# xxlong0/ESTDepth

Measured on AMD Instinct MI355X. Metric: depth frames/sec (seq_len=5, 480x640, D=64), higher is better.
Workload: dtype f32; 1 GPU; cfg2: seq_len=5, 480x640, ndepths=64, ResNet-50, Joint mode steady state (carried memory, EST on); launch=hipGraph replay, pipeline=False, graph_memory=zero-copy, conv3d_arith=f32, conv2d_arith=f32, conv3d_algo_32to32=wino3, full=False, parallelism=1 sequence per GPU

## Files before the change

### estdepth_amd/_native.py

```python
import ctypes
import os

_HERE = os.path.dirname(os.path.abspath(__file__))
LIB_PATH = os.environ.get("ESTD_LIB", os.path.join(_HERE, "lib", "libestd_hip.so"))

c_float_p = ctypes.c_void_p
c_stream = ctypes.c_void_p


class Conv3dDesc(ctypes.Structure):
    _fields_ = [
        ("N", ctypes.c_int), ("D", ctypes.c_int), ("H", ctypes.c_int), ("W", ctypes.c_int),
        ("cin_main", ctypes.c_int), ("in_stride", ctypes.c_int), ("n_tiles", ctypes.c_int),
        ("in_main", ctypes.c_void_p), ("in_extra", ctypes.c_void_p),
        ("w_main", ctypes.c_void_p), ("w_extra", ctypes.c_void_p), ("w_xout", ctypes.c_void_p),
        ("scale", ctypes.c_void_p), ("shift", ctypes.c_void_p),
        ("act_a", ctypes.c_int), ("act_b", ctypes.c_int), ("act_split", ctypes.c_int),
        ("out_main", ctypes.c_void_p), ("out_stride", ctypes.c_int), ("out_channels", ctypes.c_int),
        ("residual", ctypes.c_void_p), ("residual2", ctypes.c_void_p), ("out_scale", ctypes.c_float), ("accumulate", ctypes.c_int),
        ("out_extra", ctypes.c_void_p),
        ("head_w", ctypes.c_void_p), ("head_b", ctypes.c_void_p), ("out_head", ctypes.c_void_p),
        ("stats_partials", ctypes.c_void_p),
        ("w_split", ctypes.c_void_p),
        ("w_wino", ctypes.c_void_p),
# ... 16 lines not shown
        ("relu_before_residual", ctypes.c_int), ("relu_after_residual", ctypes.c_int),
        ("residual", ctypes.c_void_p), ("out", ctypes.c_void_p), ("w_split", ctypes.c_void_p), ("w_wino", ctypes.c_void_p),
    ]


class Conv1x1Desc(ctypes.Structure):
    _fields_ = [
        ("N", ctypes.c_int), ("H", ctypes.c_int), ("W", ctypes.c_int), ("cin", ctypes.c_int), ("cout", ctypes.c_int),
        ("stride", ctypes.c_int), ("relu", ctypes.c_int),
        ("in_", ctypes.c_void_p), ("w", ctypes.c_void_p), ("scale", ctypes.c_void_p), ("shift", ctypes.c_void_p),
        ("residual", ctypes.c_void_p), ("out", ctypes.c_void_p),
    ]


class Conv2dTapsDesc(ctypes.Structure):
    _fields_ = [
        ("N", ctypes.c_int), ("H", ctypes.c_int), ("W", ctypes.c_int), ("cin", ctypes.c_int), ("cout", ctypes.c_int),
        ("ksize", ctypes.c_int), ("stride", ctypes.c_int), ("pad", ctypes.c_int), ("relu", ctypes.c_int),
        ("in_", ctypes.c_void_p), ("w", ctypes.c_void_p), ("scale", ctypes.c_void_p), ("shift", ctypes.c_void_p),
        ("residual", ctypes.c_void_p), ("out", ctypes.c_void_p),
    ]


TSDF_MAX_FRAMES = 8
CONSISTENCY_MAX_SOURCES = 8


class TsdfIntegrateDesc(ctypes.Structure):
    _fields_ = [
        ("Z", ctypes.c_int), ("Y", ctypes.c_int), ("X", ctypes.c_int), ("T", ctypes.c_int), ("H", ctypes.c_int), ("W", ctypes.c_int),
        ("weighted", ctypes.c_int), ("no_skip", ctypes.c_int),
        ("trunc", ctypes.c_float), ("z_near", ctypes.c_float), ("conf_min", ctypes.c_float), ("w_max", ctypes.c_float),
        ("tsdf", ctypes.c_void_p), ("weight", ctypes.c_void_p),
        ("depth", ctypes.c_void_p * TSDF_MAX_FRAMES), ("conf", ctypes.c_void_p * TSDF_MAX_FRAMES), ("mats", (ctypes.c_float * 12) * TSDF_MAX_FRAMES),
    ]


class TsdfIntegrateColorDesc(ctypes.Structure):
    _fields_ = TsdfIntegrateDesc._fields_ + [("color", ctypes.c_void_p), ("image", ctypes.c_void_p * TSDF_MAX_FRAMES)]


class TsdfRaycastDesc(ctypes.Structure):
    _fields_ = [
        ("Z", ctypes.c_int), ("Y", ctypes.c_int), ("X", ctypes.c_int), ("H", ctypes.c_int), ("W", ctypes.c_int), ("n_steps", ctypes.c_int),
        ("t_min", ctypes.c_float), ("dt", ctypes.c_float), ("w_min", ctypes.c_float),
        ("tsdf", ctypes.c_void_p), ("weight", ctypes.c_void_p),
        ("depth", ctypes.c_void_p), ("normal", ctypes.c_void_p), ("out_weight", ctypes.c_void_p), ("stats", ctypes.c_void_p),
        ("mat", ctypes.c_float * 12),
    ]


class TsdfRaycastColorDesc(ctypes.Structure):
    _fields_ = TsdfRaycastDesc._fields_ + [("color", ctypes.c_void_p), ("out_color", ctypes.c_void_p)]


class DepthConsistencyDesc(ctypes.Structure):
    _fields_ = [
        ("H", ctypes.c_int), ("W", ctypes.c_int), ("S", ctypes.c_int),
        ("px_max", ctypes.c_float), ("rel_max", ctypes.c_float), ("z_near", ctypes.c_float),
        ("target", ctypes.c_void_p), ("source", ctypes.c_void_p * CONSISTENCY_MAX_SOURCES),
        ("views", ctypes.c_void_p), ("visible", ctypes.c_void_p), ("depth", ctypes.c_void_p), ("rel_err", ctypes.c_void_p),
        ("mats", ((ctypes.c_float * 12) * 2) * CONSISTENCY_MAX_SOURCES),
    ]


class CloudNearestDesc(ctypes.Structure):
    _fields_ = [
        ("M", ctypes.c_longlong), ("N", ctypes.c_longlong),
        ("query", ctypes.c_void_p), ("order", ctypes.c_void_p), ("records", ctypes.c_void_p), ("cell_start", ctypes.c_void_p),
        ("dist", ctypes.c_void_p), ("index", ctypes.c_void_p), ("stats", ctypes.c_void_p),
        ("lo", ctypes.c_float * 3), ("cell", ctypes.c_float), ("max_dist", ctypes.c_float), ("dims", ctypes.c_int * 3),
    ]


class MeshNearestDesc(ctypes.Structure):
    _fields_ = [
        ("M", ctypes.c_longlong), ("B", ctypes.c_longlong), ("P", ctypes.c_longlong),
        ("query", ctypes.c_void_p), ("order", ctypes.c_void_p), ("big_records", ctypes.c_void_p), ("records", ctypes.c_void_p),
        ("cell_start", ctypes.c_void_p), ("dist", ctypes.c_void_p), ("face", ctypes.c_void_p), ("bary", ctypes.c_void_p),
        ("closest", ctypes.c_void_p),
        ("lo", ctypes.c_float * 3), ("cell", ctypes.c_float), ("max_dist", ctypes.c_float), ("dims", ctypes.c_int * 3),
    ]


class FrameAlignDesc(ctypes.Structure):
    _fields_ = [
        ("H", ctypes.c_int), ("W", ctypes.c_int), ("Hm", ctypes.c_int), ("Wm", ctypes.c_int),
        ("dist_max", ctypes.c_float), ("z_near", ctypes.c_float), ("conf_min", ctypes.c_float),
        ("depth", ctypes.c_void_p), ("conf", ctypes.c_void_p), ("m_depth", ctypes.c_void_p), ("m_normal", ctypes.c_void_p),
        ("residual", ctypes.c_void_p), ("match", ctypes.c_void_p), ("sums", ctypes.c_void_p), ("partials", ctypes.c_void_p),
        ("L", ctypes.c_float * 12), ("Fm", ctypes.c_float * 12), ("Bm", ctypes.c_float * 12),
    ]


class RigidSystemDesc(ctypes.Structure):
    _fields_ = [
        ("N", ctypes.c_longlong), ("Nt", ctypes.c_longlong), ("Nn", ctypes.c_longlong),
        ("metric", ctypes.c_int), ("by_index", ctypes.c_int), ("two_sided", ctypes.c_int),
        ("dist_max", ctypes.c_float), ("cos_min", ctypes.c_float),
        ("moved", ctypes.c_void_p), ("moved_normal", ctypes.c_void_p), ("index", ctypes.c_void_p), ("target", ctypes.c_void_p),
        ("normal", ctypes.c_void_p), ("residual", ctypes.c_void_p), ("match", ctypes.c_void_p), ("sums", ctypes.c_void_p),
        ("partials", ctypes.c_void_p),
    ]


_SIGNATURES = {
    "estd_version": (ctypes.c_int, []),
    "estd_status_string": (ctypes.c_char_p, [ctypes.c_int]),
    "estd_profile_mark": (ctypes.c_int, [ctypes.c_int, c_stream]),
    "estd_set_reserved_cus": (ctypes.c_int, [ctypes.c_int]),
    "estd_get_reserved_cus": (ctypes.c_int, []),
    "estd_cam_pair_proj": (ctypes.c_int, [c_float_p, c_float_p, c_float_p, c_stream]),
    "estd_cam_sweep_proj": (ctypes.c_int, [c_float_p, c_float_p, c_float_p, c_float_p, c_stream]),
    "estd_cam_volume_mats": (ctypes.c_int, [c_float_p, c_float_p, c_float_p, c_float_p, c_stream]),
    "estd_homo_warping": (ctypes.c_int, [c_float_p, c_float_p, c_float_p, c_float_p,
                                         ctypes.c_int, ctypes.c_int, ctypes.c_int, ctypes.c_int, c_stream]),
    "estd_homo_warping_px": (ctypes.c_int, [c_float_p, c_float_p, c_float_p, c_float_p,
                                            ctypes.c_int, ctypes.c_int, ctypes.c_int, ctypes.c_int, c_stream]),
    "estd_warp_volume_ex": (ctypes.c_int, [c_float_p, c_float_p, c_float_p, ctypes.POINTER(WarpVolumeOpts), c_float_p,
                                           ctypes.c_int, ctypes.c_int, ctypes.c_int, ctypes.c_int, c_stream]),
    "estd_mix1x1_chw_to_hwc": (ctypes.c_int, [c_float_p, c_float_p, c_float_p, c_float_p,
                                              ctypes.c_int, ctypes.c_int, ctypes.c_int, c_stream]),
    "estd_homo_warp_costvol": (ctypes.c_int, [c_float_p, c_float_p, c_float_p, c_float_p, c_float_p,
                                              ctypes.c_int, ctypes.c_int, ctypes.c_int, c_stream]),
    "estd_conv3d_k3": (ctypes.c_int, [ctypes.POINTER(Conv3dDesc), c_stream]),
    "estd_conv3d_k3_split": (ctypes.c_int, [ctypes.POINTER(Conv3dDesc), c_stream]),
    "estd_conv3d_k3_wino": (ctypes.c_int, [ctypes.POINTER(Conv3dDesc), c_stream]),
    "estd_conv3d_k3_wino2": (ctypes.c_int, [ctypes.POINTER(Conv3dDesc), c_stream]),
    "estd_conv3d_k3_wino2x": (ctypes.c_int, [ctypes.POINTER(Conv3dDesc), c_stream]),
    "estd_conv3d_k3_wino3": (ctypes.c_int, [ctypes.POINTER(Conv3dDesc), c_stream]),
    "estd_conv3d_k3_xout": (ctypes.c_int, [ctypes.POINTER(Conv3dDesc), c_stream]),
    "estd_conv2d_k3": (ctypes.c_int, [ctypes.POINTER(Conv2dDesc), c_stream]),
    "estd_conv2d_k3_split": (ctypes.c_int, [ctypes.POINTER(Conv2dDesc), c_stream]),
    "estd_conv2d_k3_wino": (ctypes.c_int, [ctypes.POINTER(Conv2dDesc), c_stream]),
    "estd_conv2d_k3_wino2": (ctypes.c_int, [ctypes.POINTER(Conv2dDesc), c_stream]),
    "estd_conv3d_k3_grid": (ctypes.c_int, [ctypes.c_int, ctypes.c_int, ctypes.c_int, ctypes.c_int]),
    "estd_groupnorm_finalize": (ctypes.c_int, [c_float_p, ctypes.c_int, ctypes.c_double, ctypes.c_float,
                                               c_float_p, c_stream]),
    "estd_softargmin_up": (ctypes.c_int, [c_float_p, c_float_p, c_float_p, c_float_p,
                                          ctypes.c_int, ctypes.c_int, ctypes.c_int, ctypes.c_int, ctypes.c_int, c_stream]),
    "estd_warp_volume": (ctypes.c_int, [c_float_p, c_float_p, c_float_p, ctypes.c_float, ctypes.c_float, c_float_p,
                                        ctypes.c_int, ctypes.c_int, ctypes.c_int, ctypes.c_int, c_stream]),
    "estd_warp_attention": (ctypes.c_int, [c_float_p, ctypes.POINTER(ctypes.c_void_p), c_float_p, ctypes.c_int,
                                           c_float_p, ctypes.c_float, ctypes.c_float, c_float_p,
                                           ctypes.c_int, ctypes.c_int, ctypes.c_int, c_stream]),
    "estd_attention_prewarped": (ctypes.c_int, [c_float_p, ctypes.POINTER(ctypes.c_void_p), ctypes.c_int, c_float_p,
                                                ctypes.c_int64, c_stream]),
    "estd_gru_reset_apply": (ctypes.c_int, [c_float_p, c_float_p, c_float_p, c_float_p, c_float_p, c_float_p,
                                            ctypes.c_int64, c_stream]),
    "estd_gru_blend": (ctypes.c_int, [c_float_p] * 10 + [ctypes.c_int, ctypes.c_int64, c_stream]),
    "estd_bn_act_nhwc": (ctypes.c_int, [c_float_p, c_float_p, c_float_p, c_float_p, ctypes.c_int, ctypes.c_int64, ctypes.c_int, c_stream]),
    "estd_conv1x1_nhwc": (ctypes.c_int, [ctypes.POINTER(Conv1x1Desc), c_stream]),
    "estd_conv2d_taps_nhwc": (ctypes.c_int, [ctypes.POINTER(Conv2dTapsDesc), c_stream]),
    "estd_stem7x7s2_nhwc": (ctypes.c_int, [c_float_p, c_float_p, c_float_p, c_float_p, c_float_p, ctypes.c_int, ctypes.c_int, ctypes.c_int, c_stream]),
    "estd_maxpool3x3s2_nhwc": (ctypes.c_int, [c_float_p, c_float_p] + [ctypes.c_int] * 4 + [c_stream]),
    "estd_avgpool_nhwc": (ctypes.c_int, [c_float_p, c_float_p] + [ctypes.c_int] * 5 + [c_stream]),
    "estd_conv2d_small_nhwc": (ctypes.c_int, [c_float_p, c_float_p, c_float_p, c_float_p, c_float_p] + [ctypes.c_int] * 8 + [c_stream]),
    "estd_conv2d_k3_to16_nhwc": (ctypes.c_int, [c_float_p, c_float_p, c_float_p, c_float_p, c_float_p, ctypes.c_int, ctypes.c_int, ctypes.c_int,
                                                ctypes.c_int, ctypes.c_int, c_stream]),
    "estd_normalise_nhwc": (ctypes.c_int, [c_float_p, c_float_p, ctypes.c_int, ctypes.c_int64, c_stream]),
    "estd_stem3x3s2_nhwc": (ctypes.c_int, [c_float_p, c_float_p, c_float_p, c_float_p, c_float_p, ctypes.c_int, ctypes.c_int, ctypes.c_int, c_stream]),
    "estd_nhwc_to_planes": (ctypes.c_int, [c_float_p, ctypes.c_int, c_float_p, ctypes.c_int, ctypes.c_int64, c_stream]),
    "estd_planes_cat_nhwc": (ctypes.c_int, [c_float_p, ctypes.c_int, c_float_p, ctypes.c_int, ctypes.c_int, c_float_p, ctypes.c_int, ctypes.c_int64, c_stream]),
    "estd_upsample2_cat_nhwc": (ctypes.c_int, [c_float_p, ctypes.c_int, c_float_p, ctypes.c_int, c_float_p, ctypes.c_int, ctypes.c_int, ctypes.c_int, c_stream]),
    "estd_disp_head_nhwc": (ctypes.c_int, [c_float_p, c_float_p, c_float_p, ctypes.c_float, c_float_p, ctypes.c_int, ctypes.c_int, ctypes.c_int, ctypes.c_int,
                                           ctypes.c_int, c_stream]),
    "estd_spp_upsample_cat": (ctypes.c_int, [c_float_p, ctypes.c_int, c_float_p, ctypes.c_int, ctypes.POINTER(ctypes.c_void_p),
                                             ctypes.POINTER(ctypes.c_int), ctypes.POINTER(ctypes.c_int), ctypes.c_int, ctypes.c_int,
                                             c_float_p, ctypes.c_int, ctypes.c_int, ctypes.c_int, c_stream]),
    "estd_cdhw_to_vol": (ctypes.c_int, [c_float_p, c_float_p, ctypes.c_int, ctypes.c_int64, ctypes.c_int, ctypes.c_int, c_stream]),
    "estd_vol_to_cdhw": (ctypes.c_int, [c_float_p, c_float_p, ctypes.c_int, ctypes.c_int64, ctypes.c_int, ctypes.c_int, c_stream]),
    "estd_tsdf_integrate": (ctypes.c_int, [ctypes.POINTER(TsdfIntegrateDesc), c_stream]),
    "estd_tsdf_extract_points": (ctypes.c_int, [c_float_p, c_float_p, ctypes.c_int, ctypes.c_int, ctypes.c_int, ctypes.c_float,
                                                ctypes.POINTER(ctypes.c_float), ctypes.c_float, ctypes.c_void_p, ctypes.c_longlong,
                                                c_float_p, c_float_p, c_float_p, ctypes.c_void_p, c_stream]),
    "estd_tsdf_raycast": (ctypes.c_int, [ctypes.POINTER(TsdfRaycastDesc), c_stream]),
    "estd_tsdf_integrate_color": (ctypes.c_int, [ctypes.POINTER(TsdfIntegrateColorDesc), c_stream]),
    "estd_tsdf_edge_colors": (ctypes.c_int, [c_float_p, c_float_p, ctypes.c_int, ctypes.c_int, ctypes.c_int, ctypes.c_void_p, ctypes.c_longlong,
                                             c_float_p, c_stream]),
    "estd_tsdf_raycast_color": (ctypes.c_int, [ctypes.POINTER(TsdfRaycastColorDesc), c_stream]),
    "estd_depth_consistency": (ctypes.c_int, [ctypes.POINTER(DepthConsistencyDesc), c_stream]),
    "estd_cloud_cell_keys": (ctypes.c_int, [c_float_p, ctypes.c_longlong, ctypes.POINTER(ctypes.c_float), ctypes.c_float,
                                            ctypes.POINTER(ctypes.c_int), ctypes.c_void_p, c_stream]),
    "estd_cloud_nearest": (ctypes.c_int, [ctypes.POINTER(CloudNearestDesc), c_stream]),
    "estd_cloud_cell_centroids": (ctypes.c_int, [c_float_p, c_float_p, ctypes.c_int, ctypes.c_longlong, ctypes.c_void_p, ctypes.c_void_p,
                                                 ctypes.c_longlong, c_float_p, c_float_p, c_stream]),
    "estd_frame_align_partials": (ctypes.c_longlong, [ctypes.c_int, ctypes.c_int]),
    "estd_frame_align": (ctypes.c_int, [ctypes.POINTER(FrameAlignDesc), c_stream]),
    "estd_tsdf_mesh_vertices": (ctypes.c_int, [c_float_p, c_float_p, c_float_p, ctypes.c_int, ctypes.c_int, ctypes.c_int, ctypes.c_float,
                                               ctypes.POINTER(ctypes.c_float), ctypes.c_float, ctypes.c_void_p, ctypes.c_longlong,
                                               ctypes.c_void_p, c_float_p, c_float_p, c_float_p, c_float_p, c_stream]),
    "estd_tsdf_mesh_faces": (ctypes.c_int, [c_float_p, c_float_p, ctypes.c_int, ctypes.c_int, ctypes.c_int, ctypes.c_float, ctypes.c_void_p,
                                            ctypes.c_longlong, ctypes.c_void_p, ctypes.c_void_p, c_stream]),
    "estd_mesh_components": (ctypes.c_int, [ctypes.c_void_p, ctypes.c_longlong, ctypes.c_longlong, ctypes.c_void_p, ctypes.c_void_p,
                                            ctypes.c_void_p, c_stream]),
    "estd_mesh_face_area": (ctypes.c_int, [ctypes.c_void_p, ctypes.c_longlong, ctypes.c_void_p, ctypes.c_longlong, ctypes.c_void_p,
                                           ctypes.c_void_p, ctypes.c_void_p, c_stream]),
    "estd_mesh_sample": (ctypes.c_int, [ctypes.c_void_p, ctypes.c_longlong, ctypes.c_void_p, ctypes.c_longlong, ctypes.c_void_p, ctypes.c_int,
                                        ctypes.c_void_p, ctypes.c_void_p, ctypes.c_longlong, ctypes.c_longlong, ctypes.c_longlong,
                                        ctypes.c_ulonglong] + [ctypes.c_void_p] * 5 + [c_stream]),
    "estd_mesh_raster": (ctypes.c_int, [ctypes.c_void_p, ctypes.c_longlong, ctypes.c_void_p, ctypes.c_longlong, ctypes.c_longlong, ctypes.c_longlong,
                                        ctypes.POINTER(ctypes.c_double), ctypes.c_int, ctypes.c_int, ctypes.c_float, ctypes.c_int, ctypes.c_void_p,
                                        ctypes.c_void_p, c_stream]),
    "estd_mesh_raster_resolve": (ctypes.c_int, [ctypes.c_void_p, ctypes.c_longlong, ctypes.c_void_p, ctypes.c_longlong, ctypes.POINTER(ctypes.c_double),
                                                ctypes.c_int, ctypes.c_int] + [ctypes.c_void_p] * 5 + [c_stream]),
    "estd_mesh_tri_bins": (ctypes.c_int, [ctypes.c_void_p, ctypes.c_longlong, ctypes.c_void_p, ctypes.c_longlong, ctypes.POINTER(ctypes.c_float),
                                          ctypes.c_float, ctypes.POINTER(ctypes.c_int), ctypes.c_int, ctypes.c_void_p, ctypes.c_void_p,
                                          ctypes.c_void_p, c_stream]),
    "estd_mesh_tri_fill": (ctypes.c_int, [ctypes.c_void_p, ctypes.c_longlong, ctypes.c_void_p, ctypes.c_longlong, ctypes.POINTER(ctypes.c_float),
                                          ctypes.c_float, ctypes.POINTER(ctypes.c_int), ctypes.c_int, ctypes.c_void_p, ctypes.c_longlong,
                                          ctypes.c_void_p, ctypes.c_void_p, c_stream]),
    "estd_mesh_nearest": (ctypes.c_int, [ctypes.POINTER(MeshNearestDesc), c_stream]),
    "estd_mesh_cluster_faces": (ctypes.c_int, [ctypes.c_void_p, ctypes.c_longlong, ctypes.c_longlong, ctypes.c_void_p, ctypes.c_longlong,
                                               ctypes.c_void_p, ctypes.c_void_p, ctypes.c_void_p, c_stream]),
    "estd_mesh_cluster_quadrics": (ctypes.c_int, [ctypes.c_void_p, ctypes.c_longlong, ctypes.c_void_p, ctypes.c_longlong, ctypes.c_void_p,
                                                  ctypes.c_void_p, ctypes.c_void_p, ctypes.c_longlong, ctypes.c_void_p,
                                                  ctypes.POINTER(ctypes.c_float), ctypes.c_float, ctypes.POINTER(ctypes.c_int), ctypes.c_double,
                                                  ctypes.c_void_p, ctypes.c_void_p, ctypes.c_void_p, c_stream]),
    "estd_rigid_apply": (ctypes.c_int, [ctypes.c_void_p, ctypes.c_void_p, ctypes.c_longlong, ctypes.POINTER(ctypes.c_float), ctypes.c_void_p,
                                        ctypes.c_void_p, c_stream]),
    "estd_rigid_system_partials": (ctypes.c_longlong, [ctypes.c_longlong]),
    "estd_rigid_system": (ctypes.c_int, [ctypes.POINTER(RigidSystemDesc), c_stream]),
}

AB_SYMBOLS = ("estd_conv3d_k3_split", "estd_conv3d_k3_wino", "estd_conv2d_k3_split", "estd_conv2d_k3_wino", "estd_conv3d_k3_wino2x")
EXPORTED_SYMBOLS = tuple(k for k in _SIGNATURES if k not in AB_SYMBOLS)

_lib = None


def lib():
    global _lib
    if _lib is None:
        if not os.path.exists(LIB_PATH):
            raise RuntimeError("libestd_hip.so not found at %s -- build it with `python -m estdepth_amd.build` "
                               "(there is no CPU/eager fallback)" % LIB_PATH)
        handle = ctypes.CDLL(LIB_PATH)
        for name, (res, args) in _SIGNATURES.items():
            if name in AB_SYMBOLS and not hasattr(handle, name):
                continue
            fn = getattr(handle, name)
            fn.restype = res
            fn.argtypes = args
        _lib = handle
    return _lib


def has_ab():
    return all(hasattr(lib(), n) for n in AB_SYMBOLS)


def require_ab(what):
    if not has_ab():
        raise RuntimeError("%s needs the A/B kernels: rebuild the library with ESTD_BUILD_AB=1 (python -m estdepth_amd.build)" % what)


def check(status, what):
    if status != 0:
        msg = lib().estd_status_string(status).decode()
        raise RuntimeError("%s failed: %s (estd_status %d)" % (what, msg, status))
```

### estdepth_amd/backbones.py

```python
import os

import numpy as np
import torch
import torch.nn as nn
import torch.nn.functional as F


SPP_FUSED = os.environ.get("ESTD_SPP_FUSED", "1") == "1"


def conv_bn2d(cin, cout, k, stride, pad, dilation):
    return nn.Sequential(
        nn.Conv2d(cin, cout, k, stride, dilation if dilation > 1 else pad, dilation, bias=False),
        nn.BatchNorm2d(cout))


def _folded(bn):
    from . import packing
    key = (bn.weight.device, bn.weight._version, bn.bias._version, bn.running_mean._version, bn.running_var._version,
           bn.weight.data_ptr())
    c = bn.__dict__.get("_estd_fold")
    if c is None or c[0] != key:
        sc, sh = packing.fold_bn_fp32(bn, list(range(bn.num_features)))
        c = (key, sc.to(bn.weight.device), sh.to(bn.weight.device))
        bn.__dict__["_estd_fold"] = c
    return c[1], c[2]


def fused_on(mod, x):
    return mod.__dict__.get("_fuse_bn", False) and x.is_cuda and not mod.training


def conv1x1_gemm(conv, x):
    key = (conv.weight.device, conv.weight._version, conv.weight.data_ptr())
    c = conv.__dict__.get("_estd_w2")
    if c is None or c[0] != key:
        c = (key, conv.weight.detach().reshape(conv.out_channels, conv.in_channels).t().contiguous())
        conv.__dict__["_estd_w2"] = c
    if conv.stride != (1, 1):
        x = x[:, :, ::conv.stride[0], ::conv.stride[1]]
    x = x.contiguous(memory_format=torch.channels_last)
    n, cin, h, w = x.shape
    y = torch.mm(x.permute(0, 2, 3, 1).reshape(n * h * w, cin), c[1])
    if conv.bias is not None:
        y = y + conv.bias
    return y.view(n, h, w, conv.out_channels).permute(0, 3, 1, 2)


HIP_STEM = os.environ.get("ESTD_HIP_STEM", "1") == "1"
HIP_STEM7 = os.environ.get("ESTD_HIP_STEM7", "1") == "1"
HIP_POOL = os.environ.get("ESTD_HIP_POOL", "1") == "1"
GEMM_EPILOGUE = os.environ.get("ESTD_GEMM_EPILOGUE", "1") == "1"
HIP_1X1 = os.environ.get("ESTD_HIP_1X1", "all")


def _hip_1x1_wanted(conv, residual):
    if HIP_1X1 == "all" or HIP_1X1 == "1":
        return True
    if HIP_1X1 != "auto":
        return False
    return residual is not None or (conv.stride == (2, 2) and conv.in_channels <= 512) or (conv.in_channels <= 64 and conv.out_channels <= 64)


def conv1x1_bn_gemm(conv, bn, x, relu):
    key = (conv.weight.device, conv.weight._version, conv.weight.data_ptr(), bn.weight._version, bn.bias._version,
           bn.running_mean._version, bn.running_var._version)
    c = conv.__dict__.get("_estd_w2bn")
    if c is None or c[0] != key:
        sc, sh = _folded(bn)
        w2 = conv.weight.detach().reshape(conv.out_channels, conv.in_channels).t() * sc[None, :]
        c = (key, w2.contiguous(), sh.contiguous())
        conv.__dict__["_estd_w2bn"] = c
    if conv.stride != (1, 1):
        x = x[:, :, ::conv.stride[0], ::conv.stride[1]]
    x = x.contiguous(memory_format=torch.channels_last)
    n, cin, h, w = x.shape
    x2 = x.permute(0, 2, 3, 1).reshape(n * h * w, cin)
    y = torch._addmm_activation(c[2], x2, c[1], use_gelu=False) if relu else torch.addmm(c[2], x2, c[1])
    return y.view(n, h, w, conv.out_channels).permute(0, 3, 1, 2)


HIP_TAPS = os.environ.get("ESTD_HIP_TAPS", "1") == "1"


def _fits_32bit(x, conv):
    n, _, h, w = x.shape
    ho, wo = (h + conv.stride[0] - 1) // conv.stride[0], (w + conv.stride[1] - 1) // conv.stride[1]
    return max(n * h * w * conv.in_channels, n * ho * wo * conv.out_channels) * 4 < 0x7fffff00


def _hip_taps_ok(conv):
    k = conv.kernel_size[0]
    return HIP_TAPS and conv.kernel_size == (k, k) and k in (3, 5) and conv.stride in ((1, 1), (2, 2)) and conv.dilation == (1, 1) \
        and conv.groups == 1 and conv.bias is None and conv.padding[0] == conv.padding[1] and conv.in_channels % 16 == 0 \
        and conv.out_channels % 32 == 0 and conv.weight.is_cuda and conv.padding_mode == "zeros"


def _is_1x1(conv):
    return conv.kernel_size == (1, 1) and conv.padding == (0, 0) and conv.groups == 1 and conv.dilation == (1, 1)


HIP_3X3_MIN_ITEMS = int(os.environ.get("ESTD_HIP3X3_MIN_ITEMS", "128"))


def _hip_3x3_plan(conv, bn, x, relu, has_residual):
    if not conv.__dict__.get("_hip3x3", False) or conv.kernel_size != (3, 3) or conv.stride != (1, 1) or conv.groups != 1:
        return None
    if conv.bias is not None or conv.dilation not in ((1, 1), (2, 2)) or conv.padding != conv.dilation:
        return None
    if conv.in_channels % 32 or conv.out_channels % 32:
        return None
    n, _, h, w = x.shape
    if n * ((h + 7) // 8) * ((w + 15) // 16) * (conv.out_channels // 32) < HIP_3X3_MIN_ITEMS:
        return None
    from . import ops
    key = (conv.weight.device, conv.weight._version, conv.weight.data_ptr(), bn.weight._version, bn.bias._version,
           bn.running_mean._version, bn.running_var._version, relu, has_residual)
    c = conv.__dict__.get("_estd_plan3x3")
    if c is None or c[0] != key:
        c = (key, ops.Conv2dPlan(conv, bn, relu_before=relu and not has_residual, relu_after=relu and has_residual))
        conv.__dict__["_estd_plan3x3"] = c
    return c[1]


def enable_hip_3x3(root, enable=True):
    for m in root.modules():
        if isinstance(m, nn.Conv2d):
            m.__dict__["_hip3x3"] = bool(enable)
    return root


def conv_bn_act(conv, bn, x, relu, residual=None):
    from . import ops
    plan = _hip_3x3_plan(conv, bn, x, relu, residual is not None)
    if plan is not None:
        xn = x.contiguous(memory_format=torch.channels_last).permute(0, 2, 3, 1)
        rn = residual.contiguous(memory_format=torch.channels_last).permute(0, 2, 3, 1) if residual is not None else None
        return plan.run(xn, residual=rn).permute(0, 3, 1, 2)
    if _is_1x1(conv) and conv.bias is None and conv.stride in ((1, 1), (2, 2)) and conv.in_channels % 16 == 0 \
            and conv.out_channels % 32 == 0 and _hip_1x1_wanted(conv, residual) and _fits_32bit(x, conv):
        key = (conv.weight.device, conv.weight._version, conv.weight.data_ptr())
        c = conv.__dict__.get("_estd_w1x1")
        if c is None or c[0] != key:
            c = (key, conv.weight.detach().reshape(conv.out_channels, conv.in_channels).contiguous())
            conv.__dict__["_estd_w1x1"] = c
        sc, sh = _folded(bn)
        xn = x.contiguous(memory_format=torch.channels_last).permute(0, 2, 3, 1)
        rn = residual.contiguous(memory_format=torch.channels_last).permute(0, 2, 3, 1) if residual is not None else None
        return ops.conv1x1_nhwc(xn, c[1], sc, sh, conv.stride[0], relu, rn).permute(0, 3, 1, 2)
    if _hip_taps_ok(conv) and _fits_32bit(x, conv):
        from . import packing
        key = (conv.weight.device, conv.weight._version, conv.weight.data_ptr())
        c = conv.__dict__.get("_estd_wtaps")
        if c is None or c[0] != key:
            c = (key, packing.pack_conv2d_taps(conv.weight).to(conv.weight.device))
            conv.__dict__["_estd_wtaps"] = c
        sc, sh = _folded(bn)
        xn = x.contiguous(memory_format=torch.channels_last).permute(0, 2, 3, 1)
        rn = residual.contiguous(memory_format=torch.channels_last).permute(0, 2, 3, 1) if residual is not None else None
        return ops.conv2d_taps_nhwc(xn, c[1], sc, sh, conv.kernel_size[0], conv.stride[0], conv.padding[0], relu, rn).permute(0, 3, 1, 2)
    if GEMM_EPILOGUE and residual is None and _is_1x1(conv) and conv.bias is None:
        return conv1x1_bn_gemm(conv, bn, x, relu)
    y = conv1x1_gemm(conv, x) if _is_1x1(conv) else conv(x)
    if not y.is_contiguous(memory_format=torch.channels_last):
        y = y.contiguous(memory_format=torch.channels_last)
    if residual is not None and not residual.is_contiguous(memory_format=torch.channels_last):
        residual = residual.contiguous(memory_format=torch.channels_last)
    sc, sh = _folded(bn)
    return ops.bn_act_nhwc_(y, sc, sh, relu, residual)


HIP_SMALL = os.environ.get("ESTD_HIP_SMALL_CONVS", "1") == "1"


def small_conv_nhwc(conv, bn, x_nhwc, relu):
    from . import ops, packing
    k, s = conv.kernel_size[0], conv.stride[0]
    if not HIP_SMALL or conv.bias is not None or conv.groups != 1 or conv.dilation != (1, 1) or conv.kernel_size != (k, k) \
            or conv.stride != (s, s) or conv.padding != (k // 2, k // 2) or (conv.in_channels, k, s) not in ops.SMALL_CONV_SHAPES \
            or conv.out_channels % 16 or not x_nhwc.is_cuda:
        return None
    key = (conv.weight.device, conv.weight._version, conv.weight.data_ptr()) + \
        ((bn.weight._version, bn.bias._version, bn.running_mean._version, bn.running_var._version) if bn is not None else ())
    c = conv.__dict__.get("_estd_small")
    if c is None or c[0] != key:
        dev = conv.weight.device
        if bn is not None:
            sc, sh = _folded(bn)
        else:
            sc, sh = torch.ones(conv.out_channels, device=dev), torch.zeros(conv.out_channels, device=dev)
        c = (key, packing.pack_conv2d_small(conv.weight).to(dev), sc.float().contiguous(), sh.float().contiguous())
        conv.__dict__["_estd_small"] = c
    return ops.conv2d_small_nhwc(x_nhwc.contiguous(), c[1], c[2], c[3], conv.out_channels, k, s, relu)


def enable_fused_bn(root, enable=True):
    for m in root.modules():
        if isinstance(m, (_PSMBlock, PSMFeatures, _Basic, _Bottleneck, SemanticEncoder, UpBlock)):
            m.__dict__["_fuse_bn"] = bool(enable)
    return root


class _PSMBlock(nn.Module):
    def __init__(self, cin, cout, stride, downsample, pad, dilation):
        super().__init__()
        self.conv1 = nn.Sequential(conv_bn2d(cin, cout, 3, stride, pad, dilation), nn.ReLU(inplace=True))
        self.conv2 = conv_bn2d(cout, cout, 3, 1, pad, dilation)
        self.downsample = downsample

    def shortcut(self, x):
        if self.downsample is None:
            return x
        if fused_on(self, x):
            return conv_bn_act(self.downsample[0], self.downsample[1], x, relu=False)
        return self.downsample(x)

    def first(self, x):
        if fused_on(self, x):
            return conv_bn_act(self.conv1[0][0], self.conv1[0][1], x, relu=True)
        return self.conv1(x)

    def forward(self, x):
        if fused_on(self, x):
            return conv_bn_act(self.conv2[0], self.conv2[1], self.first(x), relu=False, residual=self.shortcut(x))
        y = self.conv2(self.conv1(x))
        return y + (x if self.downsample is None else self.downsample(x))


class PSMFeatures(nn.Module):

    def __init__(self):
        super().__init__()
        self._cin = 32
        self.firstconv = nn.Sequential(
            conv_bn2d(3, 32, 3, 2, 1, 1), nn.ReLU(inplace=True),
            conv_bn2d(32, 32, 3, 1, 1, 1), nn.ReLU(inplace=True),
            conv_bn2d(32, 32, 3, 1, 1, 1), nn.ReLU(inplace=True))
        self.layer1 = self._stage(32, 3, 1, 1, 1)
        self.layer2 = self._stage(64, 16, 2, 1, 1)
        self.layer3 = self._stage(128, 3, 1, 1, 1)
        self.layer4 = self._stage(128, 3, 1, 1, 2)
        for i, p in zip((1, 2, 3, 4), (32, 16, 8, 4)):
            setattr(self, "branch%d" % i, nn.Sequential(
                nn.AvgPool2d((p, p), stride=(p, p)), conv_bn2d(128, 32, 1, 1, 0, 1), nn.ReLU(inplace=True)))
        self.lastconv = nn.Sequential(conv_bn2d(320, 128, 3, 1, 1, 1), nn.ReLU(inplace=True),
                                      nn.Conv2d(128, 32, 1, 1, 0, bias=False))
        self.out_channels = [32]

    def _stage(self, planes, blocks, stride, pad, dilation):
        down = None
        if stride != 1 or self._cin != planes:
            down = nn.Sequential(nn.Conv2d(self._cin, planes, 1, stride, bias=False), nn.BatchNorm2d(planes))
        layers = [_PSMBlock(self._cin, planes, stride, down, pad, dilation)]
        self._cin = planes
        layers += [_PSMBlock(planes, planes, 1, None, pad, dilation) for _ in range(1, blocks)]
        return nn.Sequential(*layers)

    def use_hip_convs(self, enable=True):
        self._hip = bool(enable)
        self._hip_plans = None
        if enable:
            self.to(memory_format=torch.channels_last)
        return self

    def _plans(self):
        from . import ops
        key = tuple((p.data_ptr(), p._version) for p in self.parameters())
        if getattr(self, "_hip_plans", None) is None or self._hip_plans[0] != key:
            plans = {}
            fc = self.firstconv
            plans["first1"] = ops.Conv2dPlan(fc[2][0], fc[2][1], relu_before=True)
            plans["first2"] = ops.Conv2dPlan(fc[4][0], fc[4][1], relu_before=True)
            for lname in ("layer1", "layer2", "layer3", "layer4"):
                for bi, blk in enumerate(getattr(self, lname)):
                    c1 = blk.conv1[0]
                    if c1[0].stride == (1, 1):
                        plans[(lname, bi, 1)] = ops.Conv2dPlan(c1[0], c1[1], relu_before=True)
                    plans[(lname, bi, 2)] = ops.Conv2dPlan(blk.conv2[0], blk.conv2[1])
            plans["last"] = ops.Conv2dPlan(self.lastconv[0][0], self.lastconv[0][1], relu_before=True)
            self._hip_plans = (key, plans)
        return self._hip_plans[1]

    @staticmethod
    def _nhwc(t):
        return t.contiguous(memory_format=torch.channels_last).permute(0, 2, 3, 1)

    @staticmethod
    def _nchw(t):
        return t.permute(0, 3, 1, 2)

    def _forward_hip(self, x):
        P = self._plans()
        fc = self.firstconv
        x = x.contiguous(memory_format=torch.channels_last)
        c0 = fc[0][0]
        if HIP_STEM and c0.in_channels == 3 and c0.out_channels == 32 and c0.kernel_size == (3, 3) and c0.stride == (2, 2) \
                and c0.padding == (1, 1) and c0.dilation == (1, 1) and c0.bias is None:
            from . import ops
            key = (c0.weight.data_ptr(), c0.weight._version, c0.weight.device)
            cw = c0.__dict__.get("_estd_w_nchw")
            if cw is None or cw[0] != key:
                cw = (key, c0.weight.detach().contiguous(memory_format=torch.contiguous_format).clone())
                c0.__dict__["_estd_w_nchw"] = cw
            sc, sh = _folded(fc[0][1])
            x = ops.stem3x3s2_nhwc(self._nhwc(x), cw[1], sc, sh)
        else:
            x = conv_bn_act(c0, fc[0][1], x, relu=True) if fused_on(self, x) else fc[1](fc[0](x))
            x = self._nhwc(x)
        x = P["first2"].run(P["first1"].run(x))
        for lname in ("layer1", "layer2", "layer3", "layer4"):
            for bi, blk in enumerate(getattr(self, lname)):
                if (lname, bi, 1) in P:
                    y = P[(lname, bi, 1)].run(x)
# ... 240 lines not shown
```

### estdepth_amd/build.py

```python
import os
import subprocess
import sys
from concurrent.futures import ThreadPoolExecutor

HERE = os.path.dirname(os.path.abspath(__file__))
ROOT = os.path.dirname(HERE)
CSRC = os.path.join(HERE, "csrc")
OUT_DIR = os.path.join(HERE, "lib")
OBJ_DIR = os.path.join(OUT_DIR, "obj" + os.environ.get("ESTD_LIB_SUFFIX", ""))
LIB = os.path.join(OUT_DIR, "libestd_hip%s.so" % os.environ.get("ESTD_LIB_SUFFIX", ""))
SOURCES = ["conv3d_mfma.hip", "conv3d_wino2.hip", "conv3d_wino3.hip", "conv3d_xout.hip", "conv3d_wino2_c16.hip", "conv2d_mfma.hip", "conv2d_wino2.hip",
           "plane_sweep.hip", "est_fusion.hip", "refine2d.hip", "conv1x1.hip", "conv2d_taps.hip", "tsdf.hip", "tsdf_raycast.hip",
           "depth_consistency.hip", "cloud_nn.hip", "track/frame_align.hip", "track/rigid_align.hip",
           "mesh/tsdf_mesh.hip", "mesh/mesh_components.hip",
           "mesh/mesh_sample.hip", "mesh/mesh_raster.hip", "mesh/mesh_distance.hip", "mesh/mesh_simplify.hip"]
AB_SOURCES = ["conv3d_wino.hip", "conv3d_split_bf16.hip", "conv2d_wino.hip", "conv2d_split_bf16.hip", "conv3d_wino2x.hip"]
BUILD_AB = os.environ.get("ESTD_BUILD_AB", "0") == "1"
if BUILD_AB:
    SOURCES = SOURCES + AB_SOURCES
HEADERS = [os.path.join(ROOT, "include", "estd_hip.h"), os.path.join(CSRC, "estd_common.h"), os.path.join(CSRC, "estd_device.h")]
FLAGS = ["--offload-arch=gfx950", "-O3", "-std=c++17", "-fPIC",
         "-I" + os.path.join(ROOT, "include"), "-I" + CSRC] + (["-DESTD_BUILD_AB=1"] if BUILD_AB else [])
MODE_STAMP = os.path.join(OUT_DIR, ".build_mode" + os.environ.get("ESTD_LIB_SUFFIX", ""))


def _hipcc():
    for c in (os.environ.get("HIPCC"), "/opt/rocm/bin/hipcc", "hipcc"):
        if c and (os.path.isabs(c) and os.path.exists(c) or not os.path.isabs(c)):
            return c
    return "hipcc"


def _stale(target, deps):
    if not os.path.exists(target):
        return True
    t = os.path.getmtime(target)
    return any(os.path.getmtime(d) > t for d in deps)


def build(force=False, verbose=False):
    os.makedirs(OBJ_DIR, exist_ok=True)
    hipcc = _hipcc()
    mode = "ab" if BUILD_AB else "default"
    relink = (open(MODE_STAMP).read().strip() if os.path.exists(MODE_STAMP) else "default" if os.path.exists(LIB) else "") != mode
    jobs = []
    objs = []
    for src in SOURCES:
        s = os.path.join(CSRC, src)
        o = os.path.join(OBJ_DIR, src.replace(".hip", ".o"))
        os.makedirs(os.path.dirname(o), exist_ok=True)
        objs.append(o)
        if force or _stale(o, [s] + HEADERS):
            cmd = [hipcc] + FLAGS + os.environ.get("ESTD_BUILD_DEFS", "").split() + (["-Rpass-analysis=kernel-resource-usage"] if verbose else []) + ["-c", s, "-o", o]
            jobs.append(cmd)

    def run(cmd):
        r = subprocess.run(cmd, capture_output=True, text=True)
        if r.returncode != 0:
            raise RuntimeError("hipcc failed: %s\n%s" % (" ".join(cmd), r.stderr))
        return r.stderr

    if jobs:
        with ThreadPoolExecutor(max_workers=len(jobs)) as ex:
            for log in ex.map(run, jobs):
                if verbose and log:
                    sys.stderr.write(log)
    if force or jobs or relink or _stale(LIB, objs):
        run([hipcc, "--offload-arch=gfx950", "-shared", "-fPIC"] + objs + ["-o", LIB])
    build_torch_ops(force=force or relink)
    open(MODE_STAMP, "w").write(mode)
    return LIB


TORCH_OPS_SRC = os.path.join(CSRC, "torch_ops.cpp")
TORCH_OPS_LIB = os.path.join(OUT_DIR, "libestd_torch_ops%s.so" % os.environ.get("ESTD_LIB_SUFFIX", ""))


def build_torch_ops(force=False):
    if not (force or _stale(TORCH_OPS_LIB, [TORCH_OPS_SRC, HEADERS[0], LIB])):
        return TORCH_OPS_LIB
    import torch
    from torch.utils import cpp_extension
    tlib = os.path.join(os.path.dirname(torch.__file__), "lib")
    cmd = [_hipcc(), "-O2", "-std=c++17", "-fPIC", "-shared", "-D__HIP_PLATFORM_AMD__=1", "-DUSE_ROCM=1", "-DHIPBLAS_V2",
           "-D_GLIBCXX_USE_CXX11_ABI=%d" % int(torch._C._GLIBCXX_USE_CXX11_ABI), "-I" + os.path.join(ROOT, "include")] \
        + (["-DESTD_BUILD_AB=1"] if BUILD_AB else [])
    cmd += ["-I" + p for p in cpp_extension.include_paths("cuda")]
    cmd += [TORCH_OPS_SRC, "-o", TORCH_OPS_LIB, "-L" + OUT_DIR, "-l:" + os.path.basename(LIB), "-L" + tlib,
            "-lc10", "-lc10_hip", "-ltorch_cpu", "-ltorch_hip", "-ltorch", "-Wl,-rpath,$ORIGIN", "-Wl,-rpath," + tlib]
    r = subprocess.run(cmd, capture_output=True, text=True)
    if r.returncode != 0:
        raise RuntimeError("hipcc failed: %s\n%s" % (" ".join(cmd), r.stderr[-4000:]))
    return TORCH_OPS_LIB


if __name__ == "__main__":
    print(build(force="--force" in sys.argv, verbose="--verbose" in sys.argv))
```

### estdepth_amd/csrc/conv2d_taps.hip

```cpp
#include <hip/hip_runtime.h>
#include <stdint.h>
#include <stdlib.h>

#include "estd_hip.h"
#include "estd_common.h"
#include "estd_device.h"

namespace {

template <int TM, int TN, int PF, int SK>
__global__ __launch_bounds__(256) void conv2d_taps_kernel(const estd_conv2d_taps_desc p, int Ho, int Wo, int tiles_m, int tiles_n)
{
    __shared__ float4 red[SK > 1 ? (SK - 1) * TN * TM * 64 : 1];
    const int lane = threadIdx.x & 63;
    const int wave = __builtin_amdgcn_readfirstlane(threadIdx.x >> 6);
    const int g = lane >> 4, i = lane & 15;
    const int wt = SK > 1 ? (int)blockIdx.x : (int)blockIdx.x * 4 + wave;
    if (wt >= tiles_m * tiles_n) return;
    const int tn = wt % tiles_n, tm = wt / tiles_n;
    const int m0 = tm * 16 * TM, n0 = tn * 16 * TN;
    const int Mtot = p.N * Ho * Wo;
    const int cin = p.cin, cout = p.cout, ks = p.ksize;

    const __amdgpu_buffer_rsrc_t rs_x = make_rsrc_bytes(p.in, (size_t)p.N * p.H * p.W * cin * 4);
    const __amdgpu_buffer_rsrc_t rs_w = make_rsrc_bytes(p.w, (size_t)ks * ks * cout * cin * 4);
    int xbase[TM];
    unsigned xmask[TM], woff[TN];
#pragma unroll
    for (int t = 0; t < TM; ++t) {
        const int m = m0 + 16 * t + i;
        const int x = m % Wo, r = m / Wo;
        const int y = r % Ho, n = r / Ho;
        const int y0 = y * p.stride - p.pad, x0 = x * p.stride - p.pad;
        xbase[t] = (((n * p.H + y0) * p.W + x0) * cin + 4 * g) * 4;
        unsigned mk = 0;
        if (m < Mtot)
            for (int ky = 0; ky < ks; ++ky)
                for (int kx = 0; kx < ks; ++kx)
                    if ((unsigned)(y0 + ky) < (unsigned)p.H && (unsigned)(x0 + kx) < (unsigned)p.W) mk |= 1u << (ky * ks + kx);
        xmask[t] = mk;
    }
#pragma unroll
    for (int t = 0; t < TN; ++t) woff[t] = (unsigned)((n0 + 16 * t + i) * cin + 4 * g) * 4u;

    f32x4 acc[TN][TM];
#pragma unroll
    for (int a = 0; a < TN; ++a)
#pragma unroll
        for (int b = 0; b < TM; ++b) acc[a][b] = (f32x4){0.f, 0.f, 0.f, 0.f};

    const int cpt = cin >> 4;
    const int nchunks = ks * ks * cpt / SK;
    const int kbase = SK > 1 ? wave * nchunks : 0;
    int l_tap = kbase / cpt, l_kc = kbase - l_tap * cpt;
    int l_ky = l_tap / ks, l_kx = l_tap - l_ky * ks;

    float4 xq[PF][TM], wq[PF][TN];
    auto load_next = [&](float4 (&xd)[TM], float4 (&wd)[TN]) {
        const int xdelta = ((l_ky * p.W + l_kx) * cin + l_kc * 16) * 4;
        const int wdelta = (l_tap * cout * cin + l_kc * 16) * 4;
#pragma unroll
        for (int t = 0; t < TN; ++t) wd[t] = as_float4(__builtin_amdgcn_raw_buffer_load_b128(rs_w, woff[t], wdelta, 0));
#pragma unroll
        for (int t = 0; t < TM; ++t) {
            const unsigned off = ((xmask[t] >> l_tap) & 1u) ? (unsigned)(xbase[t] + xdelta) : OOB_OFFSET;
            xd[t] = as_float4(__builtin_amdgcn_raw_buffer_load_b128(rs_x, off, 0, 0));
        }
        if (++l_kc == cpt) {
            l_kc = 0; ++l_tap;
            if (++l_kx == ks) { l_kx = 0; ++l_ky; }
        }
    };
    auto mfma_chunk = [&](const float4 (&xs)[TM], const float4 (&ws)[TN]) {
#pragma unroll
        for (int e = 0; e < 4; ++e)
#pragma unroll
            for (int a = 0; a < TN; ++a) {
                const float wv = e == 0 ? ws[a].x : e == 1 ? ws[a].y : e == 2 ? ws[a].z : ws[a].w;
#pragma unroll
                for (int b = 0; b < TM; ++b) {
                    const float xv = e == 0 ? xs[b].x : e == 1 ? xs[b].y : e == 2 ? xs[b].z : xs[b].w;
                    acc[a][b] = __builtin_amdgcn_mfma_f32_16x16x4f32(wv, xv, acc[a][b], 0, 0, 0);
                }
            }
    };
#pragma unroll
    for (int j = 0; j < PF - 1; ++j)
        if (j < nchunks) load_next(xq[j], wq[j]);
    for (int c = 0; c < nchunks; c += PF) {
#pragma unroll
        for (int j = 0; j < PF; ++j) {
            const int cc = c + j;
            if (cc + PF - 1 < nchunks) load_next(xq[(j + PF - 1) % PF], wq[(j + PF - 1) % PF]);
            if (cc < nchunks) mfma_chunk(xq[j], wq[j]);
        }
    }
    if (SK > 1) {
        if (wave > 0) {
#pragma unroll
            for (int a = 0; a < TN; ++a)
#pragma unroll
                for (int b = 0; b < TM; ++b)
                    red[(((wave - 1) * TN + a) * TM + b) * 64 + lane] = make_float4(acc[a][b][0], acc[a][b][1], acc[a][b][2], acc[a][b][3]);
        }
        __syncthreads();
        if (wave > 0) return;
#pragma unroll
        for (int w = 0; w < SK - 1; ++w)
#pragma unroll
            for (int a = 0; a < TN; ++a)
#pragma unroll
                for (int b = 0; b < TM; ++b) {
                    const float4 r = red[((w * TN + a) * TM + b) * 64 + lane];
                    acc[a][b] += (f32x4){r.x, r.y, r.z, r.w};
                }
    }

    const __amdgpu_buffer_rsrc_t rs_o = make_rsrc_bytes(p.out, (size_t)Mtot * cout * 4);
    const __amdgpu_buffer_rsrc_t rs_r = make_rsrc_bytes(p.residual ? p.residual : p.out, (size_t)Mtot * cout * 4);
    const float floor_ = p.relu ? 0.0f : ESTD_NO_FLOOR;
#pragma unroll
    for (int a = 0; a < TN; ++a) {
        const int cb = n0 + 16 * a + 4 * g;
        float4 sc = make_float4(1.f, 1.f, 1.f, 1.f), sh = make_float4(0.f, 0.f, 0.f, 0.f);
        if (p.scale) sc = *reinterpret_cast<const float4*>(p.scale + cb);
        if (p.shift) sh = *reinterpret_cast<const float4*>(p.shift + cb);
        unsigned ooff[TM];
        float4 res[TM];
#pragma unroll
        for (int b = 0; b < TM; ++b) {
            const int m = m0 + 16 * b + i;
            ooff[b] = m < Mtot ? (unsigned)((size_t)m * cout + cb) * 4u : OOB_OFFSET;
        }
        if (p.residual) {
#pragma unroll
            for (int b = 0; b < TM; ++b) res[b] = as_float4(__builtin_amdgcn_raw_buffer_load_b128(rs_r, ooff[b], 0, 0));
        }
#pragma unroll
        for (int b = 0; b < TM; ++b) {
            float4 v;
            v.x = fmaf(acc[a][b][0], sc.x, sh.x); v.y = fmaf(acc[a][b][1], sc.y, sh.y);
            v.z = fmaf(acc[a][b][2], sc.z, sh.z); v.w = fmaf(acc[a][b][3], sc.w, sh.w);
            if (p.residual) { v.x += res[b].x; v.y += res[b].y; v.z += res[b].z; v.w += res[b].w; }
            v.x = fmaxf(v.x, floor_); v.y = fmaxf(v.y, floor_); v.z = fmaxf(v.z, floor_); v.w = fmaxf(v.w, floor_);
            u32x4 bits;
            __builtin_memcpy(&bits, &v, 16);
            __builtin_amdgcn_raw_buffer_store_b128(bits, rs_o, ooff[b], 0, 0);
        }
    }
}

template <int TM, int TN, int PF, int SK>
int launch_taps(const estd_conv2d_taps_desc& d, int Ho, int Wo, hipStream_t stream)
{
    const long long Mtot = (long long)d.N * Ho * Wo;
    const int tiles_m = (int)((Mtot + 16 * TM - 1) / (16 * TM)), tiles_n = d.cout / (16 * TN);
    const long long wts = (long long)tiles_m * tiles_n;
    const unsigned grid = SK > 1 ? (unsigned)wts : (unsigned)((wts + 3) / 4);
    hipLaunchKernelGGL((conv2d_taps_kernel<TM, TN, PF, SK>), dim3(grid), dim3(256), 0, stream, d, Ho, Wo, tiles_m, tiles_n);
    return ESTD_LAUNCH_CHECK();
}

constexpr int STEM_ROWS = 8;
__global__ __launch_bounds__(256) void stem7x7s2_nhwc_kernel(const float* __restrict__ in, const float* __restrict__ wpk, const float* __restrict__ scale,
                                                             const float* __restrict__ shift, float* __restrict__ out, int N, int H, int W, int Ho,
                                                             int Wo, int strips_y, int segs_x)
{
    const int lane = threadIdx.x & 63, g = lane >> 4, i = lane & 15;
    const long long wid = (long long)blockIdx.x * 4 + (threadIdx.x >> 6);
    const long long nwaves = (long long)N * strips_y * segs_x;
    if (wid >= nwaves) return;
    const int seg = (int)(wid % segs_x);
    const int strip = (int)((wid / segs_x) % strips_y);
    const int n = (int)(wid / ((long long)segs_x * strips_y));

    float wr[7][6][4];
#pragma unroll
    for (int ky = 0; ky < 7; ++ky)
#pragma unroll
        for (int s = 0; s < 6; ++s)
#pragma unroll
            for (int u = 0; u < 4; ++u) wr[ky][s][u] = wpk[((ky * 6 + s) * 4 + u) * 64 + lane];
    float4 sc[4], sh[4];
#pragma unroll
    for (int u = 0; u < 4; ++u) {
        sc[u] = reinterpret_cast<const float4*>(scale + 16 * u)[g];
        sh[u] = reinterpret_cast<const float4*>(shift + 16 * u)[g];
    }
    const __amdgpu_buffer_rsrc_t rs_in =
        __builtin_amdgcn_make_buffer_rsrc(const_cast<float*>(in + (size_t)n * H * W * 3), 0, (int)((size_t)H * W * 3 * 4), 0x00020000);
    const int x = seg * 16 + i;
    const int c0 = 2 * x - 3 + 2 * g, c1 = c0 + 1;
    const unsigned off0 = (x < Wo && (unsigned)c0 < (unsigned)W) ? (unsigned)c0 * 12u : OOB_OFFSET;
    const unsigned off1 = (x < Wo && g < 3 && (unsigned)c1 < (unsigned)W) ? (unsigned)c1 * 12u : OOB_OFFSET;
    for (int r = 0; r < STEM_ROWS; ++r) {
        const int y = strip * STEM_ROWS + r;
        if (y >= Ho) break;
        f32x4 acc[4];
#pragma unroll
        for (int u = 0; u < 4; ++u) acc[u] = (f32x4){0.f, 0.f, 0.f, 0.f};
#pragma unroll
        for (int ky = 0; ky < 7; ++ky) {
            const int yy = 2 * y - 3 + ky;
            if ((unsigned)yy >= (unsigned)H) continue;
            const int rowoff = yy * W * 12;
            const u32x3 r0 = __builtin_amdgcn_raw_buffer_load_b96(rs_in, off0, rowoff, 0);
            const u32x3 r1 = __builtin_amdgcn_raw_buffer_load_b96(rs_in, off1, rowoff, 0);
            float a[6];
            __builtin_memcpy(&a[0], &r0, 12);
            __builtin_memcpy(&a[3], &r1, 12);
#pragma unroll
            for (int s = 0; s < 6; ++s)
#pragma unroll
                for (int u = 0; u < 4; ++u) acc[u] = __builtin_amdgcn_mfma_f32_16x16x4f32(wr[ky][s][u], a[s], acc[u], 0, 0, 0);
        }
        if (x < Wo) {
#pragma unroll
            for (int u = 0; u < 4; ++u) {
                float4 o;
                o.x = fmaxf(fmaf(acc[u][0], sc[u].x, sh[u].x), 0.f);
                o.y = fmaxf(fmaf(acc[u][1], sc[u].y, sh[u].y), 0.f);
                o.z = fmaxf(fmaf(acc[u][2], sc[u].z, sh[u].z), 0.f);
                o.w = fmaxf(fmaf(acc[u][3], sc[u].w, sh[u].w), 0.f);
                *reinterpret_cast<float4*>(out + (((size_t)n * Ho + y) * Wo + x) * 64 + 16 * u + 4 * g) = o;
            }
        }
    }
}

__global__ __launch_bounds__(256) void maxpool3x3s2_nhwc_kernel(const float4* __restrict__ in, float4* __restrict__ out, int N, int H, int W, int C4,
                                                                int Ho, int Wo, long long total)
{
    const long long e = (long long)blockIdx.x * 256 + threadIdx.x;
    if (e >= total) return;
    const int c = (int)(e % C4);
    const long long pix = e / C4;
    const int x = (int)(pix % Wo), y = (int)((pix / Wo) % Ho);
    const long long n = pix / ((long long)Wo * Ho);
    const float ninf = -__builtin_inff();
    float4 m = make_float4(ninf, ninf, ninf, ninf);
#pragma unroll
    for (int ky = 0; ky < 3; ++ky) {
        const int yy = 2 * y - 1 + ky;
        if ((unsigned)yy >= (unsigned)H) continue;
#pragma unroll
        for (int kx = 0; kx < 3; ++kx) {
            const int xx = 2 * x - 1 + kx;
            if ((unsigned)xx >= (unsigned)W) continue;
            const float4 v = in[((n * H + yy) * W + xx) * C4 + c];
            m.x = (v.x > m.x || v.x != v.x) ? v.x : m.x;
            m.y = (v.y > m.y || v.y != v.y) ? v.y : m.y;
            m.z = (v.z > m.z || v.z != v.z) ? v.z : m.z;
            m.w = (v.w > m.w || v.w != v.w) ? v.w : m.w;
        }
    }
    out[e] = m;
}

__global__ __launch_bounds__(256) void avgpool_nhwc_kernel(const float4* __restrict__ in, float4* __restrict__ out, int H, int W, int C4, int k,
                                                           int Ho, int Wo, long long total)
{
    const long long e = (long long)blockIdx.x * 256 + threadIdx.x;
    if (e >= total) return;
    const int c = (int)(e % C4);
    const long long pix = e / C4;
    const int x = (int)(pix % Wo), y = (int)((pix / Wo) % Ho);
    const long long n = pix / ((long long)Wo * Ho);
    float4 s = make_float4(0.f, 0.f, 0.f, 0.f);
    for (int ky = 0; ky < k; ++ky) {
        const float4* row = in + ((n * H + (long long)y * k + ky) * W + (long long)x * k) * C4 + c;
        for (int kx = 0; kx < k; ++kx) {
            const float4 v = row[(long long)kx * C4];
            s.x += v.x; s.y += v.y; s.z += v.z; s.w += v.w;
        }
    }
    const float div = (float)(k * k);
    out[e] = make_float4(s.x / div, s.y / div, s.z / div, s.w / div);
}

}

extern "C" int estd_conv2d_taps_nhwc(const estd_conv2d_taps_desc* dp, estd_stream_t s)
{
    if (!dp) return ESTD_ERR_ARG;
    const estd_conv2d_taps_desc& d = *dp;
    if (d.N <= 0 || d.H <= 0 || d.W <= 0 || !d.in || !d.w || !d.out || d.pad < 0) return ESTD_ERR_ARG;
    if (d.stride != 1 && d.stride != 2) return ESTD_ERR_UNSUPPORTED;
    if (d.ksize != 1 && d.ksize != 3 && d.ksize != 5) return ESTD_ERR_UNSUPPORTED;
    if (d.cin < 16 || (d.cin & 15) || d.cout < 32 || (d.cout & 31)) return ESTD_ERR_UNSUPPORTED;
    if (d.H + 2 * d.pad < d.ksize || d.W + 2 * d.pad < d.ksize) return ESTD_ERR_ARG;
    const int Ho = (d.H + 2 * d.pad - d.ksize) / d.stride + 1, Wo = (d.W + 2 * d.pad - d.ksize) / d.stride + 1;
    const long long Mtot = (long long)d.N * Ho * Wo;
    const int taps = d.ksize * d.ksize;
    if (((long long)d.N * d.H + d.ksize) * d.W * d.cin * 4 >= 0x7fffff00LL || Mtot * d.cout * 4 >= 0x7fffff00LL ||
        (long long)taps * d.cin * d.cout * 4 >= 0x7fffff00LL)
        return ESTD_ERR_UNSUPPORTED;
    hipStream_t stream = estd_stream(s);
    static const int cfg_env = [] { const char* e = getenv("ESTD_CTAPS_CFG"); return e ? atoi(e) : 0; }();
    const long long want = (long long)estd_device_cus() * 7 / 2;
    auto tiles = [&](int tm, int tn) { return ((Mtot + 16 * tm - 1) / (16 * tm)) * (d.cout / (16 * tn)); };
    const bool sk4 = (d.cin & 63) == 0 && (long long)taps * d.cin >= 256;
    const bool c64 = (d.cout & 63) == 0;
    int cfg = cfg_env;
    if (cfg == 0) {
        if (c64 && tiles(4, 4) >= want) cfg = 441;
        else if (tiles(4, 2) >= want) cfg = 421;
        else if (sk4 && c64 && tiles(4, 4) >= want / 4) cfg = 444;
        else if (tiles(2, 2) >= want) cfg = 221;
        else if (sk4 && c64 && tiles(2, 4) >= want / 4) cfg = 244;
        else if (sk4 && tiles(2, 2) >= want / 4) cfg = 224;
        else if (sk4) cfg = 124;
        else cfg = 121;
    }
    if ((cfg % 10) == 4 && (d.cin & 63)) cfg = cfg - 3;
    if ((cfg / 10) % 10 == 4 && !c64) cfg -= 20;
    switch (cfg) {
    case 441: return launch_taps<4, 4, 2, 1>(d, Ho, Wo, stream);
    case 421: return launch_taps<4, 2, 3, 1>(d, Ho, Wo, stream);
    case 241: return launch_taps<2, 4, 3, 1>(d, Ho, Wo, stream);
    case 221: return launch_taps<2, 2, 4, 1>(d, Ho, Wo, stream);
    case 444: return launch_taps<4, 4, 2, 4>(d, Ho, Wo, stream);
    case 424: return launch_taps<4, 2, 3, 4>(d, Ho, Wo, stream);
    case 244: return launch_taps<2, 4, 3, 4>(d, Ho, Wo, stream);
    case 224: return launch_taps<2, 2, 4, 4>(d, Ho, Wo, stream);
    case 124: return launch_taps<1, 2, 4, 4>(d, Ho, Wo, stream);
    default: return launch_taps<1, 2, 8, 1>(d, Ho, Wo, stream);
    }
}

extern "C" int estd_stem7x7s2_nhwc(const float* in, const float* w_packed, const float* scale, const float* shift, float* out, int N, int H, int W,
                                   estd_stream_t s)
{
    if (!in || !w_packed || !scale || !shift || !out || N <= 0 || H <= 0 || W <= 0) return ESTD_ERR_ARG;
    if ((long long)H * W * 12 >= 0x7fffff00LL) return ESTD_ERR_UNSUPPORTED;
    const int Ho = (H - 1) / 2 + 1, Wo = (W - 1) / 2 + 1;
    const int strips_y = (Ho + STEM_ROWS - 1) / STEM_ROWS, segs_x = (Wo + 15) / 16;
    const long long waves = (long long)N * strips_y * segs_x;
    const long long blocks = (waves + 3) / 4;
    if (blocks > 0x7fffffffLL) return ESTD_ERR_ARG;
    hipLaunchKernelGGL(stem7x7s2_nhwc_kernel, dim3((unsigned)blocks), dim3(256), 0, estd_stream(s), in, w_packed, scale, shift, out, N, H, W, Ho, Wo,
                       strips_y, segs_x);
    return ESTD_LAUNCH_CHECK();
}

extern "C" int estd_maxpool3x3s2_nhwc(const float* in, float* out, int N, int H, int W, int C, estd_stream_t s)
{
    if (!in || !out || N <= 0 || H <= 0 || W <= 0 || C <= 0 || (C & 3)) return ESTD_ERR_ARG;
    const int Ho = (H - 1) / 2 + 1, Wo = (W - 1) / 2 + 1;
    const long long total = (long long)N * Ho * Wo * (C / 4);
    const long long blocks = (total + 255) / 256;
    if (blocks > 0x7fffffffLL) return ESTD_ERR_ARG;
    hipLaunchKernelGGL(maxpool3x3s2_nhwc_kernel, dim3((unsigned)blocks), dim3(256), 0, estd_stream(s), reinterpret_cast<const float4*>(in),
                       reinterpret_cast<float4*>(out), N, H, W, C / 4, Ho, Wo, total);
    return ESTD_LAUNCH_CHECK();
}

extern "C" int estd_avgpool_nhwc(const float* in, float* out, int N, int H, int W, int C, int k, estd_stream_t s)
{
    if (!in || !out || N <= 0 || H <= 0 || W <= 0 || C <= 0 || (C & 3) || k <= 0 || k > H || k > W) return ESTD_ERR_ARG;
    const int Ho = H / k, Wo = W / k;
    const long long total = (long long)N * Ho * Wo * (C / 4);
    const long long blocks = (total + 255) / 256;
    if (blocks > 0x7fffffffLL) return ESTD_ERR_ARG;
    hipLaunchKernelGGL(avgpool_nhwc_kernel, dim3((unsigned)blocks), dim3(256), 0, estd_stream(s), reinterpret_cast<const float4*>(in),
                       reinterpret_cast<float4*>(out), H, W, C / 4, k, Ho, Wo, total);
    return ESTD_LAUNCH_CHECK();
}
```

### estdepth_amd/csrc/estd_common.h

```cpp
#ifndef ESTD_COMMON_H
#define ESTD_COMMON_H

#include <hip/hip_runtime.h>

#include "estd_hip.h"

#define ESTD_LAUNCH_CHECK() (hipGetLastError() == hipSuccess ? ESTD_OK : ESTD_ERR_LAUNCH)

static inline hipStream_t estd_stream(estd_stream_t s) { return static_cast<hipStream_t>(s); }

#define ESTD_NO_FLOOR __builtin_nanf("")

extern "C" int estd_get_reserved_cus(void);
#include <atomic>
#include <stdio.h>
static inline int estd_device_cus(void)
{
    static std::atomic<int> cus[64];
    int dev = 0;
    if (hipGetDevice(&dev) != hipSuccess) dev = 0;
    int n = 0;
    const bool cached = (unsigned)dev < 64u;
    if (cached && (n = cus[dev].load(std::memory_order_relaxed)) > 0) return n;
    if (hipDeviceGetAttribute(&n, hipDeviceAttributeMultiprocessorCount, dev) != hipSuccess || n <= 0) {
        static std::atomic<bool> warned{false};
        if (!warned.exchange(true))
            fprintf(stderr, "libestd_hip: hipDeviceGetAttribute(MultiprocessorCount) failed for device %d: persistent grids sized for 256 CUs\n", dev);
        return 256;
    }
    if (cached) cus[dev].store(n, std::memory_order_relaxed);
    return n;
}
static inline int estd_persistent_wgs(int per_cu)
{
    const int cus = estd_device_cus() - estd_get_reserved_cus();
    return (cus > 8 ? cus : 8) * per_cu;
}
static inline int estd_persistent_grid(long long total, int per_cu)
{
    const int slots = estd_persistent_wgs(per_cu);
    int grid = total < slots ? (int)total : slots;
    if (grid >= 8) grid &= ~7;
    return grid;
}

static inline bool estd_conv3d_volume_fits_rsrc(const estd_conv3d_desc& d)
{
    const long long vox = (long long)d.D * d.H * d.W;
    const int widest = d.in_stride > d.out_stride ? d.in_stride : d.out_stride;
    return vox * widest * 4 < 0x7fffff00LL;
}

static inline int estd_conv3d_readback_kind(bool res_any, bool accumulate)
{
    return (!res_any && !accumulate) ? 0 : (!res_any ? 1 : (!accumulate ? 2 : 3));
}

static inline bool finite_pos(float v) { return v > 0.f && v < __builtin_inff(); }

int estd_wino2_c16_launch(const estd_conv3d_desc& d, hipStream_t stream);

static inline int estd_ceil_div(long long a, long long b) { return (int)((a + b - 1) / b); }

template <auto Kernel>
static inline void estd_allow_dynamic_lds(int bytes)
{
    static std::atomic<unsigned long long> done{0ull};
    int dev = 0;
    if (hipGetDevice(&dev) != hipSuccess) dev = 0;
    const unsigned long long bit = 1ull << (dev & 63);
    if (!(done.load(std::memory_order_acquire) & bit)) {
        (void)hipFuncSetAttribute(reinterpret_cast<const void*>(Kernel), hipFuncAttributeMaxDynamicSharedMemorySize, bytes);
        done.fetch_or(bit, std::memory_order_release);
    }
}

#endif
```

### estdepth_amd/csrc/torch_ops.cpp

```cpp
#include <ATen/ATen.h>
#include <ATen/hip/HIPContext.h>
#include <ATen/DeviceGuard.h>
#include <c10/hip/HIPStream.h>
#include <torch/library.h>

#include <algorithm>
#include <cmath>
#include <string>
#include <type_traits>
#include <vector>

#include "estd_hip.h"

namespace {

using at::Tensor;
using OptTensor = std::optional<Tensor>;

inline estd_stream_t cur_stream() { return static_cast<estd_stream_t>(c10::hip::getCurrentHIPStream().stream()); }

struct OpScope {
    static inline thread_local const c10::Device* cur = nullptr;
    c10::OptionalDeviceGuard guard;
    c10::Device dev;
// ... 906 lines not shown
static const int32_t* check_clusters(const Tensor& cluster, int64_t n_clusters, const Tensor& faces, const char* op)
{
    const int32_t* c = lptr<int32_t>(cluster, op, "cluster", faces, -1);
    check_count(cluster.size(0), 0, 0x7fffffffLL, op, "the number of vertices");
    check_count(n_clusters, cluster.size(0) ? 1 : 0, cluster.size(0), op, "n_clusters");
    return c;
}

std::tuple<Tensor, Tensor, Tensor> mesh_cluster_faces(const Tensor& faces, const Tensor& cluster, int64_t n_clusters)
{
    const char* op = "mesh_cluster_faces";
    const int32_t* f = faces_ptr(faces, op, "faces");
    const OpScope scope(faces);
    const int32_t* c = check_clusters(cluster, n_clusters, faces, op);
    const int64_t F = faces.size(0), V = cluster.size(0);
    TORCH_CHECK(F <= 0x7fffffffLL / 3, op, ": at most ", 0x7fffffffLL / 3, " faces, got ", F);
    Tensor corner = at::empty({3 * F}, faces.options()), triple = at::empty({F, 3}, faces.options());
    Tensor counts = at::empty({2}, faces.options().dtype(at::kLong));
    check_status(estd_mesh_cluster_faces(F ? f : nullptr, (long long)F, (long long)V, V ? c : nullptr, (long long)n_clusters,
                                         F ? corner.data_ptr<int32_t>() : nullptr, F ? triple.data_ptr<int32_t>() : nullptr,
                                         reinterpret_cast<long long*>(counts.data_ptr<int64_t>()), cur_stream()), "estd_mesh_cluster_faces");
    if (F && !n_clusters) {
        corner.zero_();
        triple.fill_(-1);
        counts.select(0, 0).fill_(F);
    }
    return {corner, triple, counts};
}

std::tuple<Tensor, Tensor, Tensor> mesh_cluster_quadrics(const Tensor& xyz, const Tensor& faces, const Tensor& order, const Tensor& segments,
                                                         const Tensor& cell_key, const Tensor& mean, const Tensor& lo, double cell,
                                                         at::IntArrayRef dims, double reg)
{
    const char* op = "mesh_cluster_quadrics";
    const OpScope scope(faces);
    const MeshArg m = check_mesh(xyz, faces, op);
    TORCH_CHECK(m.F <= 0x7fffffffLL / 3, op, ": at most ", 0x7fffffffLL / 3, " faces, got ", m.F);
    const int64_t* ord = lptr(order, op, "order", faces, 3 * m.F);
    const int64_t* seg = lptr(segments, op, "segments", faces, -1);
    TORCH_CHECK(segments.size(0) >= 1 && segments.size(0) <= m.V + 1, op, ": segments must be [K + 1] with K <= ", m.V, " vertices");
    const int64_t K = segments.size(0) - 1;
    const int64_t* key = lptr(cell_key, op, "cell_key", faces, K);
    const float* mu = check_cloud(mean, op, "mean", 3);
    TORCH_CHECK(mean.size(0) == K && mean.device() == faces.device(), op, ": mean must be [", K, ",3] on the faces' device");
    check_cloud_grid(lo, cell, dims, op, ESTD_CLOUD_KEY_MAX_DIM);
    TORCH_CHECK(std::isfinite(reg) && reg >= 0, op, ": reg must be finite and not negative, got ", reg);
    Tensor out = new_f32({K, 3}, xyz), normal = new_f32({K, 3}, xyz), placed = at::empty({K}, faces.options().dtype(at::kBool));
    const int d3[3] = {(int)dims[0], (int)dims[1], (int)dims[2]};
    check_status(estd_mesh_cluster_quadrics(m.V ? m.xyz : nullptr, (long long)m.V, m.F ? m.faces : nullptr, (long long)m.F,
                                            m.F ? reinterpret_cast<const long long*>(ord) : nullptr, reinterpret_cast<const long long*>(seg),
                                            K ? reinterpret_cast<const long long*>(key) : nullptr, (long long)K, K ? mu : nullptr,
                                            lo.data_ptr<float>(), (float)cell, d3, reg, K ? out.data_ptr<float>() : nullptr,
                                            K ? normal.data_ptr<float>() : nullptr,
                                            K ? reinterpret_cast<unsigned char*>(placed.data_ptr<bool>()) : nullptr, cur_stream()),
                 "estd_mesh_cluster_quadrics");
    if (K && !m.F) {
        out.copy_(mean);
        normal.zero_();
        placed.zero_();
    }
    return {out, normal, placed};
}

Tensor warp_attention(const Tensor& kv_target, at::TensorList kv_sources, const Tensor& mats, const Tensor& depth_values,
                      double depth_min, double depth_interval)
{
    const char* op = "warp_attention";
    const OpScope scope(kv_target);
    const float* kv = map_ptr(kv_target, {-1, -1, -1, 32}, op, "kv_target");
    const int64_t D = kv_target.size(-4), H = kv_target.size(-3), W = kv_target.size(-2), n = (int64_t)kv_sources.size();
    check_count(n, 1, ESTD_MAX_ATTENTION_SOURCES, op, "kv_sources");
    const std::vector<const float*> srcs = like_ptrs(kv_sources, kv_target, op, "kv_sources");
    const float* m = floats_ptr(mats, n * 30, op, "mats");
    const float* dv = floats_ptr(depth_values, D, op, "depth_values", true);
    Tensor xh = at::empty_like(kv_target);
    ESTD_LAUNCH(estd_warp_attention, kv, srcs.data(), m, (int)n, dv, (float)depth_min, (float)depth_interval, xh.data_ptr<float>(), (int)D, (int)H,
                (int)W);
    return xh;
}

Tensor attention_prewarped(const Tensor& kv_target, at::TensorList kv_sources)
{
    const char* op = "attention_prewarped";
    const OpScope scope(kv_target);
    const int64_t n_vox = records(kv_target, op, "kv_target"), n = (int64_t)kv_sources.size();
    check_count(n, 1, ESTD_MAX_ATTENTION_SOURCES, op, "kv_sources");
    const std::vector<const float*> srcs = like_ptrs(kv_sources, kv_target, op, "kv_sources");
    Tensor xh = at::empty_like(kv_target);
    ESTD_LAUNCH(estd_attention_prewarped, kv_target.data_ptr<float>(), srcs.data(), (int)n, xh.data_ptr<float>(), n_vox);
    return xh;
}

Tensor gru_reset_apply(const Tensor& xh, const Tensor& ru, const Tensor& stats4, const Tensor& gamma_r, const Tensor& beta_r)
{
    const char* op = "gru_reset_apply";
    const OpScope scope(xh);
    const int64_t n_vox = records(xh, op, "xh");
    const float *x = xh.data_ptr<float>(), *r = floats_ptr(ru, n_vox * 32, op, "ru");
    const float *st = floats_ptr(stats4, 4, op, "stats4"), *ga = floats_ptr(gamma_r, 16, op, "gamma_r"), *be = floats_ptr(beta_r, 16, op, "beta_r");
    Tensor xrh = at::empty_like(xh);
    ESTD_LAUNCH(estd_gru_reset_apply, x, r, st, ga, be, xrh.data_ptr<float>(), n_vox);
    return xrh;
}

void gru_blend(const Tensor& xh, const Tensor& ru, const Tensor& o_raw, const Tensor& stats_ru, const Tensor& stats_o,
               const Tensor& gamma_u, const Tensor& beta_u, const Tensor& gamma_o, const Tensor& beta_o, Tensor out_value, int64_t out_stride)
{
    const char* op = "gru_blend";
    const OpScope scope(xh);
    const int64_t n_vox = records(xh, op, "xh");
    const float *x = xh.data_ptr<float>(), *r = floats_ptr(ru, n_vox * 32, op, "ru"), *o = floats_ptr(o_raw, n_vox * 16, op, "o_raw");
    const float *sr = floats_ptr(stats_ru, 4, op, "stats_ru"), *so = floats_ptr(stats_o, 4, op, "stats_o");
    const float *gu = floats_ptr(gamma_u, 16, op, "gamma_u"), *bu = floats_ptr(beta_u, 16, op, "beta_u");
    const float *go = floats_ptr(gamma_o, 16, op, "gamma_o"), *bo = floats_ptr(beta_o, 16, op, "beta_o");
    const float* out = floats_ptr(out_value, (n_vox - 1) * out_stride + 16, op, "out_value", true, true);
    ESTD_LAUNCH(estd_gru_blend, x, r, o, sr, so, gu, bu, go, bo, mut(out), (int)out_stride, n_vox);
}

Tensor bn_act_nhwc_(Tensor x, const Tensor& scale, const Tensor& shift, bool relu, const OptTensor& residual)
{
    const char* op = "bn_act_nhwc_";
    const OpScope scope(x);
    float* xp = channels_last_ptr(x, op, "x");
    const int64_t n = x.size(0), c = x.size(1), h = x.size(2), w = x.size(3);
    const float *sc = floats_ptr(scale, c, op, "scale"), *sh = floats_ptr(shift, c, op, "shift");
    const float* res = (residual.has_value() && residual->defined()) ? channels_last_ptr(*residual, op, "residual", &x) : nullptr;
    ESTD_LAUNCH(estd_bn_act_nhwc, xp, sc, sh, res, relu ? 1 : 0, n * h * w, (int)c);
    return x;
}

Tensor spp_upsample_cat(const Tensor& raw, const Tensor& skip, at::TensorList branches)
{
    const char* op = "spp_upsample_cat";
    const OpScope scope(raw);
    const float* rp = map_ptr(raw, {-1, -1, -1, -1}, op, "raw");
    const int64_t n = raw.size(-4), h = raw.size(-3), w = raw.size(-2), cr = raw.size(-1), nb = (int64_t)branches.size();
    const float* sp = map_ptr(skip, {n, h, w, -1}, op, "skip");
    const int64_t cs = skip.size(-1);
    check_count(nb, 1, 4, op, "branches");
    std::vector<const float*> ptrs(nb);
    std::vector<int> bh(nb), bw(nb);
    int64_t cb = -1;
    for (int64_t k = 0; k < nb; ++k) {
        const std::string item = "branches[" + std::to_string(k) + "]";
        ptrs[k] = map_ptr(branches[k], {n, -1, -1, cb}, op, item.c_str());
        bh[k] = (int)branches[k].size(-3); bw[k] = (int)branches[k].size(-2); cb = branches[k].size(-1);
    }
    Tensor out = new_f32({n, h, w, cr + cs + nb * cb}, raw);
    ESTD_LAUNCH(estd_spp_upsample_cat, rp, (int)cr, sp, (int)cs, ptrs.data(), bh.data(), bw.data(), (int)nb, (int)cb, out.data_ptr<float>(), (int)n,
                (int)h, (int)w);
    return out;
}

template <class Desc>
static Tensor desc_conv(const char* op, int (*launch)(const Desc*, estd_stream_t), const char* what, Desc d, const Tensor& x, const Tensor& w,
                        at::IntArrayRef w_tail, int64_t ho, int64_t wo, const OptTensor& scale, const OptTensor& shift, bool relu,
                        const OptTensor& residual)
{
    d.w = map_ptr(w, w_tail, op, "w");
    const int64_t n = x.size(-4), cout = w.size(-2);
    d.N = (int)n; d.H = (int)x.size(-3); d.W = (int)x.size(-2); d.cin = (int)x.size(-1); d.cout = (int)cout; d.relu = relu ? 1 : 0;
    d.in = x.data_ptr<float>();
    d.scale = opt_floats_ptr(scale, cout, op, "scale"); d.shift = opt_floats_ptr(shift, cout, op, "shift");
    if (residual.has_value() && residual->defined()) d.residual = map_ptr(*residual, {n, ho, wo, cout}, op, "residual");
    Tensor out = new_f32({n, ho, wo, cout}, x);
    d.out = out.data_ptr<float>();
    check_status(launch(&d, cur_stream()), what);
    return out;
}

Tensor conv1x1_nhwc(const Tensor& x, const Tensor& w2, const OptTensor& scale, const OptTensor& shift, int64_t stride, bool relu,
                    const OptTensor& residual)
{
    const char* op = "conv1x1_nhwc";
    const OpScope scope(x);
    map_ptr(x, {-1, -1, -1, -1}, op, "x");
    check_count(stride, 1, 2, op, "stride");
    estd_conv1x1_desc d{};
    d.stride = (int)stride;
    return desc_conv(op, estd_conv1x1_nhwc, "estd_conv1x1_nhwc", d, x, w2, {-1, x.size(-1)}, (x.size(-3) - 1) / stride + 1,
                     (x.size(-2) - 1) / stride + 1, scale, shift, relu, residual);
}

Tensor conv2d_taps_nhwc(const Tensor& x, const Tensor& w_taps, const OptTensor& scale, const OptTensor& shift, int64_t ksize, int64_t stride,
                        int64_t pad, bool relu, const OptTensor& residual)
{
    const char* op = "conv2d_taps_nhwc";
    const OpScope scope(x);
    map_ptr(x, {-1, -1, -1, -1}, op, "x");
    check_count(stride, 1, 2, op, "stride");
    estd_conv2d_taps_desc d{};
    d.ksize = (int)ksize; d.stride = (int)stride; d.pad = (int)pad;
    return desc_conv(op, estd_conv2d_taps_nhwc, "estd_conv2d_taps_nhwc", d, x, w_taps, {ksize * ksize, -1, x.size(-1)},
                     (x.size(-3) + 2 * pad - ksize) / stride + 1, (x.size(-2) + 2 * pad - ksize) / stride + 1, scale, shift, relu, residual);
}

template <class Launch>
static Tensor packed_conv(const char* op, const char* what, const Tensor& x, const float* w, const Tensor& scale, const Tensor& shift,
                          at::IntArrayRef out_shape, Launch launch)
{
    const float *sc = floats_ptr(scale, out_shape[3], op, "scale"), *sh = floats_ptr(shift, out_shape[3], op, "shift");
    Tensor out = new_f32(out_shape, x);
    check_status(launch(x.data_ptr<float>(), w, sc, sh, out.data_ptr<float>()), what);
    return out;
}

Tensor stem7x7s2_nhwc(const Tensor& x, const Tensor& w_packed, const Tensor& scale, const Tensor& shift)
{
    const char* op = "stem7x7s2_nhwc";
    const OpScope scope(x);
    map_ptr(x, {-1, -1, -1, 3}, op, "x");
    const int n = (int)x.size(-4), h = (int)x.size(-3), w = (int)x.size(-2);
    return packed_conv(op, "estd_stem7x7s2_nhwc", x, floats_ptr(w_packed, 7 * 6 * 4 * 64, op, "w_packed"), scale, shift,
                       {n, (h - 1) / 2 + 1, (w - 1) / 2 + 1, 64},
                       [&](auto... p) { return estd_stem7x7s2_nhwc(p..., n, h, w, cur_stream()); });
}

Tensor stem3x3s2_nhwc(const Tensor& x, const Tensor& weight, const Tensor& scale, const Tensor& shift)
{
    const char* op = "stem3x3s2_nhwc";
    const OpScope scope(x);
    map_ptr(x, {-1, -1, -1, 3}, op, "x");
    const int n = (int)x.size(-4), h = (int)x.size(-3), w = (int)x.size(-2);
    return packed_conv(op, "estd_stem3x3s2_nhwc", x, map_ptr(weight, {32, 3, 3, 3}, op, "weight"), scale, shift,
                       {n, (h - 1) / 2 + 1, (w - 1) / 2 + 1, 32},
                       [&](auto... p) { return estd_stem3x3s2_nhwc(p..., n, h, w, cur_stream()); });
}

Tensor conv2d_small_nhwc(const Tensor& x, const Tensor& w_packed, const Tensor& scale, const Tensor& shift, int64_t cout, int64_t ksize,
                         int64_t stride, bool relu)
{
    const char* op = "conv2d_small_nhwc";
    const OpScope scope(x);
    map_ptr(x, {-1, -1, -1, -1}, op, "x");
    const int64_t n = x.size(-4), h = x.size(-3), w = x.size(-2), cin = x.size(-1);
    TORCH_CHECK((ksize == 1 || ksize == 3) && (stride == 1 || stride == 2) && cout > 0 && cout % 16 == 0 && cin % 16 == 0,
                "conv2d_small_nhwc: ksize 1|3, stride 1|2, the channel counts of x and cout multiples of 16");
    const float* wp = floats_ptr(w_packed, cout / 16 * ksize * ksize * (cin / 16) * 256, op, "w_packed");
    const int64_t pad = ksize / 2;
    return packed_conv(op, "estd_conv2d_small_nhwc", x, wp, scale, shift, {n, (h + 2 * pad - ksize) / stride + 1, (w + 2 * pad - ksize) / stride + 1, cout},
                       [&](auto... p) {
                           return estd_conv2d_small_nhwc(p..., (int)n, (int)h, (int)w, (int)cin, (int)cout, (int)ksize, (int)stride, relu ? 1 : 0,
                                                         cur_stream());
                       });
}

Tensor conv2d_k3_to16_nhwc(const Tensor& x, const Tensor& w_packed, const Tensor& scale, const Tensor& shift, bool upsample)
{
    const char* op = "conv2d_k3_to16_nhwc";
    const OpScope scope(x);
    map_ptr(x, {-1, -1, -1, -1}, op, "x");
    const int64_t n = x.size(-4), c = x.size(-1), h = (upsample ? 2 : 1) * x.size(-3), w = (upsample ? 2 : 1) * x.size(-2);
    TORCH_CHECK(c == 16 || c == 32, "conv2d_k3_to16_nhwc: x must have 16 or 32 channels, got ", c);
    const float* wp = floats_ptr(w_packed, 9 * (c / 16) * 256, op, "w_packed");
    return packed_conv(op, "estd_conv2d_k3_to16_nhwc", x, wp, scale, shift, {n, h, w, 16}, [&](auto... p) {
        return estd_conv2d_k3_to16_nhwc(p..., (int)n, (int)h, (int)w, (int)c, upsample ? 1 : 0, cur_stream());
    });
}

Tensor maxpool3x3s2_nhwc(const Tensor& x)
{
    const OpScope scope(x);
    const float* xp = map_ptr(x, {-1, -1, -1, -1}, "maxpool3x3s2_nhwc", "x");
    const int64_t n = x.size(-4), h = x.size(-3), w = x.size(-2), c = x.size(-1);
    Tensor out = new_f32({n, (h - 1) / 2 + 1, (w - 1) / 2 + 1, c}, x);
    ESTD_LAUNCH(estd_maxpool3x3s2_nhwc, xp, out.data_ptr<float>(), (int)n, (int)h, (int)w, (int)c);
    return out;
}

Tensor avgpool_nhwc(const Tensor& x, int64_t k)
{
    const OpScope scope(x);
    const float* xp = map_ptr(x, {-1, -1, -1, -1}, "avgpool_nhwc", "x");
    const int64_t n = x.size(-4), h = x.size(-3), w = x.size(-2), c = x.size(-1);
    check_count(k, 1, std::min(h, w), "avgpool_nhwc", "k");
    Tensor out = new_f32({n, h / k, w / k, c}, x);
    ESTD_LAUNCH(estd_avgpool_nhwc, xp, out.data_ptr<float>(), (int)n, (int)h, (int)w, (int)c, (int)k);
    return out;
}

Tensor normalise_nhwc(const Tensor& imgs)
{
    const OpScope scope(imgs);
    const float* in = map_ptr(imgs, {-1, 3, -1, -1}, "normalise_nhwc", "imgs");
    const int64_t n = imgs.size(-4), h = imgs.size(-2), w = imgs.size(-1);
    Tensor out = new_f32({n, h, w, 3}, imgs);
    ESTD_LAUNCH(estd_normalise_nhwc, in, out.data_ptr<float>(), (int)n, h * w);
    return out;
}

Tensor nhwc_to_planes(const Tensor& x)
{
    const OpScope scope(x);
    const float* xp = map_ptr(x, {-1, -1, -1, -1}, "nhwc_to_planes", "x");
    const int64_t n = x.size(-4), h = x.size(-3), w = x.size(-2), c = x.size(-1);
    Tensor out = new_f32({n, c, h, w}, x);
    ESTD_LAUNCH(estd_nhwc_to_planes, xp, (int)c, out.data_ptr<float>(), (int)n, h * w);
    return out;
}

Tensor planes_cat_nhwc(const Tensor& a, const Tensor& b, bool relu_b)
{
    const char* op = "planes_cat_nhwc";
    const OpScope scope(a);
    const float* ap = map_ptr(a, {-1, -1, -1, -1}, op, "a");
    const int64_t n = a.size(-4), ca = a.size(-3), h = a.size(-2), w = a.size(-1);
    const float* bp = map_ptr(b, {n, -1, h, w}, op, "b");
    const int64_t cb = b.size(-3);
    Tensor out = new_f32({n, h, w, ca + cb}, a);
    ESTD_LAUNCH(estd_planes_cat_nhwc, ap, (int)ca, bp, (int)cb, relu_b ? 1 : 0, out.data_ptr<float>(), (int)n, h * w);
    return out;
}

Tensor upsample2_cat_nhwc(const Tensor& x, const Tensor& skip)
{
    const char* op = "upsample2_cat_nhwc";
    const OpScope scope(x);
    const float* xp = map_ptr(x, {-1, -1, -1, -1}, op, "x");
    const int64_t n = x.size(-4), h = 2 * x.size(-3), w = 2 * x.size(-2), cx = x.size(-1);
    const float* sp = map_ptr(skip, {n, h, w, -1}, op, "skip");
    const int64_t cs = skip.size(-1);
    Tensor out = new_f32({n, h, w, cx + cs}, x);
    ESTD_LAUNCH(estd_upsample2_cat_nhwc, xp, (int)cx, sp, (int)cs, out.data_ptr<float>(), (int)n, (int)h, (int)w);
    return out;
}

Tensor disp_head_nhwc(const Tensor& x, const Tensor& weight, const Tensor& bias, double depth_max, int64_t upscale)
{
    const char* op = "disp_head_nhwc";
    const OpScope scope(x);
    const float* xp = map_ptr(x, {-1, -1, -1, -1}, op, "x");
    const int64_t n = x.size(-4), h = x.size(-3), w = x.size(-2), c = x.size(-1);
    const float *wp = map_ptr(weight, {1, c, 3, 3}, op, "weight"), *bp = floats_ptr(bias, 1, op, "bias");
    Tensor out = new_f32({n, 1, upscale * h, upscale * w}, x);
    ESTD_LAUNCH(estd_disp_head_nhwc, xp, wp, bp, (float)depth_max, out.data_ptr<float>(), (int)n, (int)h, (int)w, (int)c, (int)upscale);
    return out;
}

void cdhw_to_vol(const Tensor& src, Tensor dst, int64_t dst_stride, int64_t dst_off)
{
    const char* op = "cdhw_to_vol";
    const OpScope scope(src);
    const float* sp = fptr(src, "src", true, op);
    TORCH_CHECK(src.dim() >= 2 && src.size(0) >= 1, op, ": src must be [C, ...] with C >= 1, got ", src.sizes());
    const int64_t C = src.size(0), S = src.numel() / C;
    check_count(dst_off, 0, dst_stride, op, "dst_off");
// ... 50 lines not shown
        }
        const int64_t n = (int64_t)P.size();
        TORCH_CHECK(n >= 2, "camera_matrices_host: the EST fusion needs at least one other view");
        const Tensor kinv = at::inverse(K);
        vol = at::empty({T, n - 1, 30}, poses.options());
        for (int64_t i = 0; i < T; ++i) {
            const Tensor inv_i = at::inverse(P[i]);
            int64_t r = 0;
            for (int64_t j = 0; j < n; ++j) {
                if (j == i) continue;
                const Tensor rel = at::matmul(P[j], inv_i);
                const Tensor m = at::inverse(rel);
                vol.index_put_({i, r, Slice(None, 9)}, kinv[0].reshape({9}));
                vol.index_put_({i, r, Slice(9, 21)}, m.index({0, Slice(None, 3), Slice()}).reshape({12}));
                vol.index_put_({i, r, Slice(21, None)}, K[0].reshape({9}));
                ++r;
            }
        }
    } else {
        vol = at::empty({0}, poses.options());
    }
    return {sweep, vol};
}

int64_t set_reserved_cus(int64_t n) { return estd_set_reserved_cus((int)n); }
std::tuple<Tensor, Tensor, Tensor> frame_align(const Tensor& depth, const OptTensor& conf, const Tensor& m_depth, const Tensor& m_normal,
                                               const Tensor& mats, double dist_max, double z_near, double conf_min)
{
    const char* op = "frame_align";
    const OpScope scope(depth);
    estd_frame_align_desc d{};
    d.depth = map_ptr(depth, {-1, -1}, op, "depth");
    const int64_t H = depth.size(-2), W = depth.size(-1);
    check_map_size(H, W, op, "depth");
    d.conf = opt_fptr(conf, "conf");
    if (d.conf) map_ptr(*conf, {H, W}, op, "conf");
    d.m_depth = map_ptr(m_depth, {-1, -1}, op, "m_depth");
    const int64_t Hm = m_depth.size(-2), Wm = m_depth.size(-1);
    check_map_size(Hm, Wm, op, "m_depth");
    d.m_normal = map_ptr(m_normal, {Hm, Wm, 3}, op, "m_normal");
    const float* m = host_values(mats, 36, op, "mats", "[3,12] (L, Fm, Bm)", true);
    d.H = (int)H; d.W = (int)W; d.Hm = (int)Hm; d.Wm = (int)Wm;
    d.dist_max = positive_square_f32(dist_max, op, "dist_max", true); d.z_near = not_negative_f32(z_near, op, "z_near");
    d.conf_min = not_nan_f32(conf_min, op, "conf_min");
    for (int i = 0; i < 12; ++i) { d.L[i] = m[i]; d.Fm[i] = m[12 + i]; d.Bm[i] = m[24 + i]; }
    Tensor residual = new_f32({H, W}, depth), match = at::empty({H, W}, depth.options().dtype(at::kInt));
    Tensor sums = at::empty({ESTD_FRAME_ALIGN_SUMS}, depth.options().dtype(at::kDouble));
    Tensor partials = at::empty({estd_frame_align_partials((int)H, (int)W) / 8}, depth.options().dtype(at::kDouble));
    d.residual = residual.data_ptr<float>(); d.match = match.data_ptr<int>();
    d.sums = sums.data_ptr<double>(); d.partials = partials.data_ptr<double>();
    check_status(estd_frame_align(&d, cur_stream()), "estd_frame_align");
    return {residual, match, sums};
}

std::tuple<Tensor, Tensor> rigid_apply(const Tensor& src, const OptTensor& src_normal, const Tensor& T)
{
    const char* op = "rigid_apply";
    const OpScope scope(src);
    const float* sp = check_cloud(src, op, "src", 3);
    const int64_t n = src.size(0);
    const bool normals = src_normal.has_value() && src_normal->defined();
    const float* np = nullptr;
    if (normals) {
        np = check_cloud(*src_normal, op, "src_normal", 3);
        TORCH_CHECK(src_normal->size(0) == n && src_normal->device() == src.device(), op, ": src_normal must be [", n, ",3] on the points' device");
    }
    const float* t = host_values(T, 12, op, "T", "[3,4]", true);
    Tensor moved = new_f32({n, 3}, src), moved_normal = new_f32({normals ? n : 0, 3}, src);
    if (n)
        check_status(estd_rigid_apply(sp, np, (long long)n, t, moved.data_ptr<float>(), normals ? moved_normal.data_ptr<float>() : nullptr, cur_stream()),
                     "estd_rigid_apply");
    return {moved, moved_normal};
}

std::tuple<Tensor, Tensor, Tensor> rigid_system(const Tensor& moved, const OptTensor& moved_normal, const Tensor& index, const Tensor& target,
                                                const OptTensor& normal, bool by_index, int64_t metric, double dist_max, double cos_min, bool two_sided)
{
    const char* op = "rigid_system";
    const OpScope scope(moved);
    estd_rigid_system_desc d{};
    d.moved = check_cloud(moved, op, "moved", 3);
    const int64_t N = moved.size(0);
    if (moved_normal.has_value() && moved_normal->defined()) {
        d.moved_normal = check_cloud(*moved_normal, op, "moved_normal", 3);
        TORCH_CHECK(moved_normal->size(0) == N && moved_normal->device() == moved.device(), op, ": moved_normal must be [", N, ",3] on the points' device");
    }
    d.index = reinterpret_cast<const long long*>(lptr(index, op, "index", moved, N));
    d.target = check_cloud(target, op, "target", 3);
    const int64_t Nt = target.size(0);
    TORCH_CHECK(target.device() == moved.device() && (by_index || Nt >= N), op, ": target must be on the points' device, and [n,3] with n >= ", N,
                " when it is not read by index");
    int64_t Nn = Nt;
    if (normal.has_value() && normal->defined()) {
        d.normal = check_cloud(*normal, op, "normal", 3);
        TORCH_CHECK(normal->device() == moved.device(), op, ": normal must be on the points' device");
        Nn = normal->size(0);
    }
    check_count(metric, ESTD_RIGID_PLANE, ESTD_RIGID_POINT, op, "metric");
    d.dist_max = positive_square_f32(dist_max, op, "dist_max", true);
    d.cos_min = d.moved_normal ? not_nan_f32(cos_min, op, "cos_min") : (float)cos_min;
    TORCH_CHECK(d.normal || !(metric == ESTD_RIGID_PLANE || (d.moved_normal && std::isfinite(d.cos_min))), op,
                ": the plane metric and the cosine gate need the target's normals");
    d.N = (long long)N; d.Nt = (long long)Nt; d.Nn = (long long)Nn;
    d.metric = (int)metric; d.by_index = by_index; d.two_sided = two_sided;
    Tensor residual = new_f32({N}, moved), match = at::empty({N}, moved.options().dtype(at::kLong));
    Tensor sums = at::empty({ESTD_RIGID_SYSTEM_SUMS}, moved.options().dtype(at::kDouble));
    Tensor partials = at::empty({estd_rigid_system_partials((long long)N) / 8}, moved.options().dtype(at::kDouble));
    d.residual = residual.data_ptr<float>(); d.match = reinterpret_cast<long long*>(match.data_ptr<int64_t>());
    d.sums = sums.data_ptr<double>(); d.partials = N ? partials.data_ptr<double>() : nullptr;
    check_status(estd_rigid_system(&d, cur_stream()), "estd_rigid_system");
    return {residual, match, sums};
}

void profile_mark(int64_t id) { check_status(estd_profile_mark((int)id, cur_stream()), "estd_profile_mark"); }
int64_t conv3d_grid(int64_t N, int64_t D, int64_t H, int64_t W)
{
    const int g = estd_conv3d_k3_grid((int)N, (int)D, (int)H, (int)W);
    check_status(g < 0 ? g : ESTD_OK, "estd_conv3d_k3_grid");
    return g;
}

}

TORCH_LIBRARY(estdepth_hip, m)
{
    m.def("cam_pair_proj(Tensor src_proj, Tensor ref_proj) -> Tensor");
    m.def("cam_sweep_proj(Tensor ref_pose, Tensor src_pose, Tensor intr) -> Tensor");
    m.def("cam_volume_mats(Tensor pose_j, Tensor? pose_i, Tensor intr, Tensor(a!) out) -> ()");
    m.def("homo_warping(Tensor src_chw, Tensor proj12, Tensor depth_values, int D) -> Tensor");
    m.def("homo_warping_px(Tensor src_chw, Tensor proj12, Tensor depth_dhw) -> Tensor");
    m.def("mix1x1(Tensor in_chw, Tensor w, Tensor? bias) -> Tensor");
    m.def("homo_warp_costvol(Tensor src_mix, Tensor ref_mix, Tensor proj12, Tensor depth_values, int D, Tensor(a!) out) -> ()");
    m.def("conv3d_k3(Tensor x, Tensor? x_extra, Tensor? w_main, Tensor? w_extra, Tensor? w_xout, Tensor? w_alt, Tensor scale, Tensor shift, "
          "int[] dims, int cin_main, int in_stride, int n_tiles, int act_a, int act_b, int act_split, Tensor(a!)? out, int out_stride, "
          "int out_channels, Tensor? residual, Tensor? residual2, float out_scale, bool accumulate, Tensor(b!)? out_extra, Tensor? head_w, "
          "Tensor? head_b, Tensor(c!)? out_head, Tensor(d!)? stats_partials, int variant, Tensor? gate_r=None, Tensor? gate_stats=None, "
          "Tensor? gate_gamma=None, Tensor? gate_beta=None) -> ()");
    m.def("conv2d_k3(Tensor x_nhwc, Tensor? w, Tensor? w_alt, Tensor scale, Tensor shift, int cout, int dilation, int group_tiles, "
          "bool relu_before_residual, bool relu_after_residual, Tensor? residual, int variant) -> Tensor");
    m.def("groupnorm_finalize(Tensor partials, int n_blocks, float count, float eps) -> Tensor");
    m.def("softargmin_up(Tensor logits, Tensor depth_values, int scale) -> (Tensor, Tensor)");
    m.def("warp_volume(Tensor vol, Tensor mats30, Tensor depth, float depth_min, float depth_interval) -> Tensor");
    m.def("warp_volume_ex(Tensor vol, Tensor mats30, Tensor depth, bool depth_per_voxel, float depth_min, float depth_interval, "
          "bool use_disp, float disp_min, float disp_interval, bool border, float padding_value) -> Tensor");
    m.def("warp_attention(Tensor kv_target, Tensor[] kv_sources, Tensor mats, Tensor depth_values, float depth_min, float depth_interval) -> Tensor");
    m.def("attention_prewarped(Tensor kv_target, Tensor[] kv_sources) -> Tensor");
    m.def("gru_reset_apply(Tensor xh, Tensor ru, Tensor stats4, Tensor gamma_r, Tensor beta_r) -> Tensor");
    m.def("gru_blend(Tensor xh, Tensor ru, Tensor o_raw, Tensor stats_ru, Tensor stats_o, Tensor gamma_u, Tensor beta_u, Tensor gamma_o, "
          "Tensor beta_o, Tensor(a!) out_value, int out_stride) -> ()");
    m.def("bn_act_nhwc_(Tensor(a!) x, Tensor scale, Tensor shift, bool relu, Tensor? residual) -> Tensor(a!)");
    m.def("spp_upsample_cat(Tensor raw, Tensor skip, Tensor[] branches) -> Tensor");
    m.def("conv1x1_nhwc(Tensor x, Tensor w, Tensor? scale, Tensor? shift, int stride, bool relu, Tensor? residual) -> Tensor");
    m.def("conv2d_taps_nhwc(Tensor x, Tensor w, Tensor? scale, Tensor? shift, int ksize, int stride, int pad, bool relu, Tensor? residual) -> Tensor");
    m.def("stem7x7s2_nhwc(Tensor x, Tensor w_packed, Tensor scale, Tensor shift) -> Tensor");
    m.def("maxpool3x3s2_nhwc(Tensor x) -> Tensor");
    m.def("avgpool_nhwc(Tensor x, int k) -> Tensor");
    m.def("conv2d_small_nhwc(Tensor x, Tensor w_packed, Tensor scale, Tensor shift, int cout, int ksize, int stride, bool relu) -> Tensor");
    m.def("conv2d_k3_to16_nhwc(Tensor x, Tensor w_packed, Tensor scale, Tensor shift, bool upsample) -> Tensor");
    m.def("normalise_nhwc(Tensor imgs) -> Tensor");
    m.def("stem3x3s2_nhwc(Tensor x, Tensor weight, Tensor scale, Tensor shift) -> Tensor");
    m.def("nhwc_to_planes(Tensor x) -> Tensor");
    m.def("planes_cat_nhwc(Tensor a, Tensor b, bool relu_b) -> Tensor");
    m.def("upsample2_cat_nhwc(Tensor x, Tensor skip) -> Tensor");
    m.def("disp_head_nhwc(Tensor x, Tensor weight, Tensor bias, float depth_max, int upscale) -> Tensor");
    m.def("cdhw_to_vol(Tensor src, Tensor(a!) dst, int dst_stride, int dst_off) -> ()");
    m.def("vol_to_cdhw(Tensor src, int C, int[] dims, int src_stride, int src_off) -> Tensor");
    m.def("camera_matrices_host(Tensor cam_poses, Tensor cam_intr, Tensor[] pre_poses, bool with_volume) -> (Tensor, Tensor)");
    m.def("tsdf_integrate_(Tensor(a!) volume, Tensor[] depths, Tensor[] confs, Tensor mats, float trunc, float z_near, float conf_min, "
          "bool weighted, float w_max, bool no_skip) -> Tensor(a!)");
    m.def("tsdf_extract_points(Tensor volume, float voxel_size, Tensor origin, float w_min, int capacity) -> (Tensor, Tensor, Tensor, Tensor, Tensor)");
    m.def("tsdf_raycast(Tensor volume, Tensor mat, int H, int W, float t_min, float dt, int n_steps, float w_min, bool stats) -> "
          "(Tensor, Tensor, Tensor, Tensor)");
    m.def("tsdf_integrate_color_(Tensor(a!) volume, Tensor(b!) color, Tensor[] depths, Tensor[] confs, Tensor[] images, Tensor mats, float trunc, "
          "float z_near, float conf_min, bool weighted, float w_max, bool no_skip) -> Tensor(a!)");
    m.def("tsdf_edge_colors(Tensor volume, Tensor color, Tensor edge) -> Tensor");
    m.def("tsdf_mesh_vertices(Tensor volume, Tensor? color, float voxel_size, Tensor origin, float w_min, int capacity) -> "
          "(Tensor, Tensor, Tensor, Tensor, Tensor, Tensor)");
    m.def("tsdf_mesh_faces(Tensor volume, float w_min, int capacity) -> (Tensor, Tensor, Tensor)");
    m.def("mesh_components(Tensor faces, int n_vertices) -> (Tensor, Tensor, Tensor)");
    m.def("mesh_face_area(Tensor xyz, Tensor faces) -> (Tensor, Tensor, Tensor)");
    m.def("mesh_sample(Tensor xyz, Tensor faces, Tensor? attrs, int n_samples, int seed) -> (Tensor, Tensor, Tensor, Tensor, Tensor, Tensor, Tensor)");
    m.def("mesh_raster(Tensor xyz, Tensor faces, Tensor mat, int H, int W, float z_near, bool preload) -> (Tensor, Tensor, Tensor, Tensor, Tensor)");
    m.def("tsdf_raycast_color(Tensor volume, Tensor color, Tensor mat, int H, int W, float t_min, float dt, int n_steps, float w_min) -> "
          "(Tensor, Tensor, Tensor, Tensor)");
    m.def("depth_consistency(Tensor target, Tensor[] sources, Tensor mats, float px_max, float rel_max, float z_near) -> "
          "(Tensor, Tensor, Tensor, Tensor)");
    m.def("cloud_cell_keys(Tensor points, Tensor lo, float cell, int[] dims) -> Tensor");
    m.def("cloud_nearest(Tensor query, Tensor order, Tensor records, Tensor cell_start, Tensor lo, float cell, int[] dims, float max_dist, "
          "bool stats) -> (Tensor, Tensor, Tensor)");
    m.def("cloud_cell_centroids(Tensor points, Tensor attrs, Tensor order, Tensor segments) -> (Tensor, Tensor)");
    m.def("mesh_tri_bins(Tensor xyz, Tensor faces, Tensor lo, float cell, int[] dims, int big_cells) -> (Tensor, Tensor, Tensor)");
    m.def("mesh_tri_fill(Tensor xyz, Tensor faces, Tensor lo, float cell, int[] dims, int big_cells, Tensor offset, int n_pairs) -> "
          "(Tensor, Tensor)");
    m.def("mesh_cluster_faces(Tensor faces, Tensor cluster, int n_clusters) -> (Tensor, Tensor, Tensor)");
    m.def("mesh_cluster_quadrics(Tensor xyz, Tensor faces, Tensor order, Tensor segments, Tensor cell_key, Tensor mean, Tensor lo, float cell, "
          "int[] dims, float reg) -> (Tensor, Tensor, Tensor)");
    m.def("mesh_nearest(Tensor query, Tensor order, Tensor big_records, Tensor records, Tensor cell_start, Tensor lo, float cell, int[] dims, "
          "float max_dist, bool bary, bool closest) -> (Tensor, Tensor, Tensor, Tensor)");
    m.def("frame_align(Tensor depth, Tensor? conf, Tensor m_depth, Tensor m_normal, Tensor mats, float dist_max, float z_near, float conf_min) -> "
          "(Tensor, Tensor, Tensor)");
    m.def("rigid_apply(Tensor src, Tensor? src_normal, Tensor T) -> (Tensor, Tensor)");
    m.def("rigid_system(Tensor moved, Tensor? moved_normal, Tensor index, Tensor target, Tensor? normal, bool by_index, int metric, float dist_max, "
          "float cos_min, bool two_sided) -> (Tensor, Tensor, Tensor)");
    m.def("profile_mark(int id) -> ()");
    m.def("set_reserved_cus(int n) -> int");
    m.def("conv3d_grid(int N, int D, int H, int W) -> int");
}

TORCH_LIBRARY_IMPL(estdepth_hip, CUDA, m)
{
    m.impl("cam_pair_proj", cam_pair_proj);
    m.impl("cam_sweep_proj", cam_sweep_proj);
    m.impl("cam_volume_mats", cam_volume_mats);
    m.impl("homo_warping", homo_warping);
    m.impl("homo_warping_px", homo_warping_px);
    m.impl("mix1x1", mix1x1);
    m.impl("homo_warp_costvol", homo_warp_costvol);
    m.impl("conv3d_k3", conv3d_k3);
    m.impl("conv2d_k3", conv2d_k3);
    m.impl("groupnorm_finalize", groupnorm_finalize);
    m.impl("softargmin_up", softargmin_up);
    m.impl("warp_volume", warp_volume);
    m.impl("warp_volume_ex", warp_volume_ex);
    m.impl("warp_attention", warp_attention);
    m.impl("attention_prewarped", attention_prewarped);
    m.impl("gru_reset_apply", gru_reset_apply);
    m.impl("gru_blend", gru_blend);
    m.impl("bn_act_nhwc_", bn_act_nhwc_);
    m.impl("spp_upsample_cat", spp_upsample_cat);
    m.impl("conv1x1_nhwc", conv1x1_nhwc);
    m.impl("conv2d_taps_nhwc", conv2d_taps_nhwc);
    m.impl("stem7x7s2_nhwc", stem7x7s2_nhwc);
    m.impl("maxpool3x3s2_nhwc", maxpool3x3s2_nhwc);
    m.impl("avgpool_nhwc", avgpool_nhwc);
    m.impl("conv2d_small_nhwc", conv2d_small_nhwc);
    m.impl("conv2d_k3_to16_nhwc", conv2d_k3_to16_nhwc);
    m.impl("normalise_nhwc", normalise_nhwc);
    m.impl("stem3x3s2_nhwc", stem3x3s2_nhwc);
    m.impl("nhwc_to_planes", nhwc_to_planes);
    m.impl("planes_cat_nhwc", planes_cat_nhwc);
    m.impl("upsample2_cat_nhwc", upsample2_cat_nhwc);
    m.impl("disp_head_nhwc", disp_head_nhwc);
    m.impl("cdhw_to_vol", cdhw_to_vol);
    m.impl("vol_to_cdhw", vol_to_cdhw);
    m.impl("tsdf_integrate_", tsdf_integrate_);
    m.impl("tsdf_extract_points", tsdf_extract_points);
    m.impl("tsdf_raycast", tsdf_raycast);
    m.impl("tsdf_integrate_color_", tsdf_integrate_color_);
    m.impl("tsdf_edge_colors", tsdf_edge_colors);
    m.impl("tsdf_mesh_vertices", tsdf_mesh_vertices);
    m.impl("tsdf_mesh_faces", tsdf_mesh_faces);
    m.impl("mesh_components", mesh_components);
    m.impl("mesh_face_area", mesh_face_area);
    m.impl("mesh_sample", mesh_sample);
    m.impl("mesh_raster", mesh_raster);
    m.impl("tsdf_raycast_color", tsdf_raycast_color);
    m.impl("depth_consistency", depth_consistency);
    m.impl("cloud_cell_keys", cloud_cell_keys);
    m.impl("cloud_nearest", cloud_nearest);
    m.impl("cloud_cell_centroids", cloud_cell_centroids);
    m.impl("mesh_tri_bins", mesh_tri_bins);
    m.impl("mesh_tri_fill", mesh_tri_fill);
    m.impl("mesh_nearest", mesh_nearest);
    m.impl("mesh_cluster_faces", mesh_cluster_faces);
    m.impl("mesh_cluster_quadrics", mesh_cluster_quadrics);
    m.impl("frame_align", frame_align);
    m.impl("rigid_apply", rigid_apply);
    m.impl("rigid_system", rigid_system);
}

TORCH_LIBRARY_IMPL(estdepth_hip, CPU, m)
{
    m.impl("camera_matrices_host", camera_matrices_host);
}

TORCH_LIBRARY_IMPL(estdepth_hip, CompositeExplicitAutograd, m)
{
    m.impl("profile_mark", profile_mark);
    m.impl("set_reserved_cus", set_reserved_cus);
    m.impl("conv3d_grid", conv3d_grid);
}
```

### estdepth_amd/ops.py

```python
import collections
import ctypes
import math
import os

import torch

from . import _native as N
from . import packing

BINDING = os.environ.get("ESTD_BINDING", "torch")
_TORCH_OPS_LIB = os.path.join(os.path.dirname(os.path.abspath(__file__)), "lib", "libestd_torch_ops.so")
_torch_ops = None


def T():
    global _torch_ops
    if _torch_ops is None:
        if BINDING not in ("torch", "ctypes"):
            raise RuntimeError("ESTD_BINDING must be 'torch' or 'ctypes', got %r" % (BINDING,))
        if not os.path.exists(_TORCH_OPS_LIB):
            raise RuntimeError("libestd_torch_ops.so not found at %s -- build it with `python -m estdepth_amd.build` "
                               "(there is no CPU/eager fallback)" % _TORCH_OPS_LIB)
        N.lib()
        torch.ops.load_library(_TORCH_OPS_LIB)
# ... 584 lines not shown
def groupnorm_finalize(partials, n_blocks, count, eps=1e-5):
    if _use_torch():
        return T().groupnorm_finalize(partials, n_blocks, float(count), float(eps))
    _need(_chk(partials, "partials", torch.float64, op="groupnorm_finalize").numel() >= n_blocks * 4,
          "groupnorm_finalize: partials must be a contiguous float64 ROCm tensor with 4 doubles per block")
    out = torch.empty(4, device=partials.device, dtype=torch.float32)
    _launch(partials.device, N.lib().estd_groupnorm_finalize, _p(partials), n_blocks, float(count), float(eps), _p(out))
    return out


def softargmin_up(logits, depth_values, scale=4):
    op = "softargmin_up"
    with _Prof("softargmin", lambda: 4.0 * (logits.numel() // logits.shape[-3]) * (logits.shape[-3] + 2 * scale * scale)):
        if _use_torch():
            return T().softargmin_up(logits, depth_values, scale)
        Nn, D, H, W = _map(logits, (-1, -1, -1, -1), op, "logits")
        dev = logits.device
        _floats(depth_values, D, op, "depth_values", dev, at_least=True)
        depth = torch.empty((Nn, 1, H * scale, W * scale), device=dev)
        prob = torch.empty_like(depth)
        _launch(dev, N.lib().estd_softargmin_up, _p(logits), _p(depth_values), _p(depth), _p(prob), Nn, D, H, W, scale)
    return depth, prob


def _warp_vol(op, entry, vol, mats30, depth, depth_per_voxel, *scalars):
    C, D, H, W = _map(vol, (-1, -1, -1, -1), op, "vol")
    dev = vol.device
    _floats(mats30, 30, op, "mats30", dev)
    _floats(depth, D * H * W if depth_per_voxel else D, op, "depth", dev, at_least=True)
    out = torch.empty_like(vol)
    _launch(dev, entry, _p(vol), _p(mats30), _p(depth), *scalars, _p(out), C, D, H, W)
    return out


def warp_volume_cdhw(vol, mats30, depth_values, depth_min, depth_interval):
    if _use_torch():
        return T().warp_volume(vol, mats30, depth_values, float(depth_min), float(depth_interval))
    return _warp_vol("warp_volume", N.lib().estd_warp_volume, vol, mats30, depth_values, False, float(depth_min), float(depth_interval))


def warp_volume_ex_cdhw(vol, mats30, depth, depth_per_voxel, depth_min, depth_interval, disp_min=None, disp_interval=None,
                        border=False, padding_value=0.0):
    use_disp = disp_min is not None
    dmin_ = float(disp_min) if use_disp else 0.0
    dint_ = float(disp_interval) if (use_disp and disp_interval is not None) else (0.0 if use_disp else 1.0)
    if _use_torch():
        return T().warp_volume_ex(vol, mats30, depth, bool(depth_per_voxel), float(depth_min), float(depth_interval), use_disp,
                                  dmin_, dint_, bool(border), float(padding_value))
    o = N.WarpVolumeOpts(int(bool(depth_per_voxel)), int(use_disp), int(bool(border)), float(depth_min), float(depth_interval),
                         dmin_, dint_, float(padding_value))
    return _warp_vol("warp_volume_ex", N.lib().estd_warp_volume_ex, vol, mats30, depth, depth_per_voxel, ctypes.byref(o))


def warp_attention(kv_target, kv_sources, mats, depth_values, depth_min, depth_interval):
    op = "warp_attention"
    kv_sources = list(kv_sources)
    with _Prof(op, lambda: 4.0 * 16 * (kv_target.numel() // 32) * (2 + 2 * len(kv_sources))):
        if _use_torch():
            return T().warp_attention(kv_target, kv_sources, mats, depth_values, float(depth_min), float(depth_interval))
        D, H, W, _ = _map(kv_target, (-1, -1, -1, 32), op, "kv_target")
        dev, n = kv_target.device, len(kv_sources)
        _count(n, 1, MAX_ATTENTION_SOURCES, op, "kv_sources")
        srcs = _like(kv_sources, kv_target, op, "kv_sources", dev)
        _floats(mats, n * 30, op, "mats", dev)
        _floats(depth_values, D, op, "depth_values", dev, at_least=True)
        xh = torch.empty_like(kv_target)
        _launch(dev, N.lib().estd_warp_attention, _p(kv_target), srcs, _p(mats), n, _p(depth_values), float(depth_min), float(depth_interval),
                _p(xh), D, H, W)
    return xh


def attention_prewarped(kv_target, kv_sources):
    kv_sources = list(kv_sources)
    if _use_torch():
        return T().attention_prewarped(kv_target, kv_sources)
    op = "attention_prewarped"
    n_vox = _records(kv_target, op, "kv_target")
    dev, n = kv_target.device, len(kv_sources)
    _count(n, 1, MAX_ATTENTION_SOURCES, op, "kv_sources")
    srcs = _like(kv_sources, kv_target, op, "kv_sources", dev)
    xh = torch.empty_like(kv_target)
    _launch(dev, N.lib().estd_attention_prewarped, _p(kv_target), srcs, n, _p(xh), n_vox)
    return xh


def gru_reset_apply(xh, ru, stats4, gamma_r, beta_r):
    op = "gru_reset_apply"
    with _Prof("gru_elementwise", lambda: 4.0 * 16 * (xh.numel() // 32) * 2):
        if _use_torch():
            return T().gru_reset_apply(xh, ru, stats4, gamma_r, beta_r)
        n_vox = _records(xh, op, "xh")
        dev = xh.device
        _floats(ru, n_vox * 32, op, "ru", dev)
        _floats(stats4, 4, op, "stats4", dev)
        _floats(gamma_r, 16, op, "gamma_r", dev)
        _floats(beta_r, 16, op, "beta_r", dev)
        xrh = torch.empty_like(xh)
        _launch(dev, N.lib().estd_gru_reset_apply, _p(xh), _p(ru), _p(stats4), _p(gamma_r), _p(beta_r), _p(xrh), n_vox)
    return xrh


def gru_blend(xh, ru, o_raw, stats_ru, stats_o, gamma_u, beta_u, gamma_o, beta_o, out_value, out_stride):
    op = "gru_blend"
    with _Prof("gru_elementwise", lambda: 4.0 * 16 * (xh.numel() // 32) * 3):
        if _use_torch():
            return T().gru_blend(xh, ru, o_raw, stats_ru, stats_o, gamma_u, beta_u, gamma_o, beta_o, out_value, out_stride)
        n_vox = _records(xh, op, "xh")
        dev = xh.device
        _floats(ru, n_vox * 32, op, "ru", dev)
        _floats(o_raw, n_vox * 16, op, "o_raw", dev)
        for name, t in (("stats_ru", stats_ru), ("stats_o", stats_o)):
            _floats(t, 4, op, name, dev)
        for name, t in (("gamma_u", gamma_u), ("beta_u", beta_u), ("gamma_o", gamma_o), ("beta_o", beta_o)):
            _floats(t, 16, op, name, dev)
        _floats(out_value, (n_vox - 1) * out_stride + 16, op, "out_value", dev, at_least=True, strided=True)
        _launch(dev, N.lib().estd_gru_blend, _p(xh), _p(ru), _p(o_raw), _p(stats_ru), _p(stats_o), _p(gamma_u), _p(beta_u), _p(gamma_o), _p(beta_o),
                _p(out_value), out_stride, n_vox)


def bn_act_nhwc_(x, scale, shift, relu, residual=None):
    if _use_torch():
        return T().bn_act_nhwc_(x, scale, shift, bool(relu), residual)
    op = "bn_act_nhwc_"
    n, c, h, w = _channels_last(x, op, "x")
    dev = x.device
    _floats(scale, c, op, "scale", dev)
    _floats(shift, c, op, "shift", dev)
    if residual is not None:
        _channels_last(residual, op, "residual", dev, like=x)
    _launch(dev, N.lib().estd_bn_act_nhwc, _p(x), _p(scale), _p(shift), _p(residual), 1 if relu else 0, n * h * w, c)
    return x


def spp_upsample_cat(raw, skip, branches):
    branches = list(branches)
    if _use_torch():
        return T().spp_upsample_cat(raw, skip, branches)
    op = "spp_upsample_cat"
    n, h, w, cr = _map(raw, (-1, -1, -1, -1), op, "raw")
    dev, nb = raw.device, len(branches)
    cs = _map(skip, (n, h, w, -1), op, "skip", dev)[3]
    _count(nb, 1, 4, op, "branches")
    bh, bw, cb = [], [], -1
    for k, b in enumerate(branches):
        _, hk, wk, cb = _map(b, (n, -1, -1, cb), op, "branches[%d]" % k, dev)
        bh.append(hk)
        bw.append(wk)
    out = torch.empty((n, h, w, cr + cs + nb * cb), device=dev)
    _launch(dev, N.lib().estd_spp_upsample_cat, _p(raw), cr, _p(skip), cs, (ctypes.c_void_p * nb)(*[b.data_ptr() for b in branches]),
            (ctypes.c_int * nb)(*bh), (ctypes.c_int * nb)(*bw), nb, cb, _p(out), n, h, w)
    return out


def _desc_conv(op, entry, d, x, w, w_tail, ho, wo, scale, shift, relu, residual):
    n, h, wd, cin = x.shape[-4:]
    dev = x.device
    cout = _map(w, w_tail, op, "w", dev)[-2]
    d.N, d.H, d.W, d.cin, d.cout, d.relu = n, h, wd, cin, cout, int(bool(relu))
    d.in_, d.w = x.data_ptr(), w.data_ptr()
    d.scale, d.shift = _p(_opt_floats(scale, cout, op, "scale", dev)), _p(_opt_floats(shift, cout, op, "shift", dev))
    if residual is not None:
        _map(residual, (n, ho, wo, cout), op, "residual", dev)
        d.residual = residual.data_ptr()
    out = torch.empty((n, ho, wo, cout), device=dev)
    d.out = out.data_ptr()
    _launch(dev, entry, ctypes.byref(d))
    return out


def conv1x1_nhwc(x, w2, scale, shift, stride=1, relu=False, residual=None):
    if _use_torch():
        return T().conv1x1_nhwc(x, w2, scale, shift, int(stride), bool(relu), residual)
    op = "conv1x1_nhwc"
    n, h, w, c = _map(x, (-1, -1, -1, -1), op, "x")
    _count(stride, 1, 2, op, "stride")
    d = N.Conv1x1Desc()
    d.stride = int(stride)
    return _desc_conv(op, N.lib().estd_conv1x1_nhwc, d, x, w2, (-1, c), (h - 1) // stride + 1, (w - 1) // stride + 1, scale, shift, relu, residual)


def conv2d_taps_nhwc(x, w_taps, scale, shift, ksize, stride=1, pad=None, relu=False, residual=None):
    pad = ksize // 2 if pad is None else pad
    if _use_torch():
        return T().conv2d_taps_nhwc(x, w_taps, scale, shift, int(ksize), int(stride), int(pad), bool(relu), residual)
    op = "conv2d_taps_nhwc"
    n, h, w, c = _map(x, (-1, -1, -1, -1), op, "x")
    _count(stride, 1, 2, op, "stride")
    d = N.Conv2dTapsDesc()
    d.ksize, d.stride, d.pad = int(ksize), int(stride), int(pad)
    return _desc_conv(op, N.lib().estd_conv2d_taps_nhwc, d, x, w_taps, (ksize * ksize, -1, c), (h + 2 * pad - ksize) // stride + 1,
                      (w + 2 * pad - ksize) // stride + 1, scale, shift, relu, residual)


def _packed_conv(op, entry, x, w, scale, shift, out_shape, *sizes):
    dev = x.device
    _floats(scale, out_shape[3], op, "scale", dev)
    _floats(shift, out_shape[3], op, "shift", dev)
    out = torch.empty(out_shape, device=dev)
    _launch(dev, entry, _p(x), _p(w), _p(scale), _p(shift), _p(out), *sizes)
    return out


def stem7x7s2_nhwc(x, w_packed, scale, shift):
    if _use_torch():
        return T().stem7x7s2_nhwc(x, w_packed, scale, shift)
    op = "stem7x7s2_nhwc"
    n, h, w, _ = _map(x, (-1, -1, -1, 3), op, "x")
    _floats(w_packed, 7 * 6 * 4 * 64, op, "w_packed", x.device)
    return _packed_conv(op, N.lib().estd_stem7x7s2_nhwc, x, w_packed, scale, shift, (n, (h - 1) // 2 + 1, (w - 1) // 2 + 1, 64), n, h, w)


def stem3x3s2_nhwc(x, weight, scale, shift):
    if _use_torch():
        return T().stem3x3s2_nhwc(x, weight, scale, shift)
    op = "stem3x3s2_nhwc"
    n, h, w, _ = _map(x, (-1, -1, -1, 3), op, "x")
    _map(weight, (32, 3, 3, 3), op, "weight", x.device)
    return _packed_conv(op, N.lib().estd_stem3x3s2_nhwc, x, weight, scale, shift, (n, (h - 1) // 2 + 1, (w - 1) // 2 + 1, 32), n, h, w)


SMALL_CONV_SHAPES = {(32, 3, 2), (32, 1, 2), (32, 1, 1), (64, 1, 1), (128, 1, 1)}


def conv2d_small_nhwc(x, w_packed, scale, shift, cout, ksize, stride, relu):
    if _use_torch():
        return T().conv2d_small_nhwc(x, w_packed, scale, shift, int(cout), int(ksize), int(stride), bool(relu))
    op = "conv2d_small_nhwc"
    n, h, w, c = _map(x, (-1, -1, -1, -1), op, "x")
    _need(ksize in (1, 3) and stride in (1, 2) and cout > 0 and cout % 16 == 0 and c % 16 == 0,
          "conv2d_small_nhwc: ksize 1|3, stride 1|2, the channel counts of x and cout multiples of 16")
    _floats(w_packed, cout // 16 * ksize * ksize * (c // 16) * 256, op, "w_packed", x.device)
    pad = ksize // 2
    return _packed_conv(op, N.lib().estd_conv2d_small_nhwc, x, w_packed, scale, shift,
                        (n, (h + 2 * pad - ksize) // stride + 1, (w + 2 * pad - ksize) // stride + 1, cout),
                        n, h, w, c, int(cout), int(ksize), int(stride), int(bool(relu)))


def conv2d_k3_to16_nhwc(x, w_packed, scale, shift, upsample=False):
    if _use_torch():
        return T().conv2d_k3_to16_nhwc(x, w_packed, scale, shift, bool(upsample))
    op = "conv2d_k3_to16_nhwc"
    n, h, w, c = _map(x, (-1, -1, -1, -1), op, "x")
    _need(c in (16, 32), "conv2d_k3_to16_nhwc: x must have 16 or 32 channels, got %d" % c)
    _floats(w_packed, 9 * (c // 16) * 256, op, "w_packed", x.device)
    u = 2 if upsample else 1
    return _packed_conv(op, N.lib().estd_conv2d_k3_to16_nhwc, x, w_packed, scale, shift, (n, u * h, u * w, 16), n, u * h, u * w, c, int(bool(upsample)))


def maxpool3x3s2_nhwc(x):
    if _use_torch():
        return T().maxpool3x3s2_nhwc(x)
    n, h, w, c = _map(x, (-1, -1, -1, -1), "maxpool3x3s2_nhwc", "x")
    out = torch.empty((n, (h - 1) // 2 + 1, (w - 1) // 2 + 1, c), device=x.device)
    _launch(x.device, N.lib().estd_maxpool3x3s2_nhwc, _p(x), _p(out), n, h, w, c)
    return out


def avgpool_nhwc(x, k):
    if _use_torch():
        return T().avgpool_nhwc(x, int(k))
    n, h, w, c = _map(x, (-1, -1, -1, -1), "avgpool_nhwc", "x")
    _count(k, 1, min(h, w), "avgpool_nhwc", "k")
    out = torch.empty((n, h // k, w // k, c), device=x.device)
    _launch(x.device, N.lib().estd_avgpool_nhwc, _p(x), _p(out), n, h, w, c, int(k))
    return out


def normalise_nhwc(imgs):
    if _use_torch():
        return T().normalise_nhwc(imgs)
    n, _, h, w = _map(imgs, (-1, 3, -1, -1), "normalise_nhwc", "imgs")
    out = torch.empty((n, h, w, 3), device=imgs.device)
    _launch(imgs.device, N.lib().estd_normalise_nhwc, _p(imgs), _p(out), n, h * w)
    return out


def nhwc_to_planes(x):
    if _use_torch():
        return T().nhwc_to_planes(x)
    n, h, w, c = _map(x, (-1, -1, -1, -1), "nhwc_to_planes", "x")
    out = torch.empty((n, c, h, w), device=x.device)
    _launch(x.device, N.lib().estd_nhwc_to_planes, _p(x), c, _p(out), n, h * w)
    return out


def planes_cat_nhwc(a, b, relu_b=False):
    if _use_torch():
        return T().planes_cat_nhwc(a, b, bool(relu_b))
    op = "planes_cat_nhwc"
    n, ca, h, w = _map(a, (-1, -1, -1, -1), op, "a")
    cb = _map(b, (n, -1, h, w), op, "b", a.device)[1]
    out = torch.empty((n, h, w, ca + cb), device=a.device)
    _launch(a.device, N.lib().estd_planes_cat_nhwc, _p(a), ca, _p(b), cb, int(bool(relu_b)), _p(out), n, h * w)
    return out


def upsample2_cat_nhwc(x, skip):
    if _use_torch():
        return T().upsample2_cat_nhwc(x, skip)
    op = "upsample2_cat_nhwc"
    n, hx, wx, cx = _map(x, (-1, -1, -1, -1), op, "x")
    h, w = 2 * hx, 2 * wx
    cs = _map(skip, (n, h, w, -1), op, "skip", x.device)[3]
    out = torch.empty((n, h, w, cx + cs), device=x.device)
    _launch(x.device, N.lib().estd_upsample2_cat_nhwc, _p(x), cx, _p(skip), cs, _p(out), n, h, w)
    return out


def disp_head_nhwc(x, weight, bias, depth_max, upscale=1):
    if _use_torch():
        return T().disp_head_nhwc(x, weight, bias, float(depth_max), int(upscale))
    op = "disp_head_nhwc"
    n, h, w, c = _map(x, (-1, -1, -1, -1), op, "x")
    _map(weight, (1, c, 3, 3), op, "weight", x.device)
    _floats(bias, 1, op, "bias", x.device)
    out = torch.empty((n, 1, upscale * h, upscale * w), device=x.device)
    _launch(x.device, N.lib().estd_disp_head_nhwc, _p(x), _p(weight), _p(bias), float(depth_max), _p(out), n, h, w, c, int(upscale))
    return out


def cdhw_to_vol(src, dst, dst_stride, dst_off):
    if _use_torch():
        return T().cdhw_to_vol(src, dst, dst_stride, dst_off)
    op = "cdhw_to_vol"
    _chk(src, "src", op=op)
    _need(src.dim() >= 2 and src.shape[0] >= 1, "%s: src must be [C, ...] with C >= 1, got %s" % (op, tuple(src.shape)))
    C = src.shape[0]
    S = src.numel() // C
    _count(dst_off, 0, dst_stride, op, "dst_off")
    _floats(dst, S * dst_stride, op, "dst", src.device, at_least=True, strided=True)
    _launch(src.device, N.lib().estd_cdhw_to_vol, _p(src), _p(dst), C, S, dst_stride, dst_off)


def vol_to_cdhw(src, C, dims, src_stride, src_off):
    dims = list(dims)
    if _use_torch():
        return T().vol_to_cdhw(src, C, dims, src_stride, src_off)
    op = "vol_to_cdhw"
    _count(len(dims), 3, 3, op, "dims")
    D, H, W = dims
    _count(src_off, 0, src_stride, op, "src_off")
    _floats(src, D * H * W * src_stride, op, "src", at_least=True, strided=True)
    out = torch.empty((C, D, H, W), device=src.device)
    _launch(src.device, N.lib().estd_vol_to_cdhw, _p(src), _p(out), C, D * H * W, src_stride, src_off)
# ... 694 lines not shown
```

### include/estd_hip.h

```cpp
#ifndef ESTD_HIP_H
#define ESTD_HIP_H

#include <stdint.h>

#ifdef __cplusplus
extern "C" {
#endif

typedef void* estd_stream_t;

enum estd_status {
    ESTD_OK = 0,
    ESTD_ERR_ARG = -1,
    ESTD_ERR_LAUNCH = -2,
    ESTD_ERR_UNSUPPORTED = -3
};

enum estd_act { ESTD_ACT_NONE = 0, ESTD_ACT_RELU = 1, ESTD_ACT_TANH = 2 };

#define ESTD_MAX_ATTENTION_SOURCES 16

int estd_version(void);
int estd_profile_mark(int id, estd_stream_t stream);
const char* estd_status_string(int status);
int estd_set_reserved_cus(int n);
int estd_get_reserved_cus(void);


int estd_cam_pair_proj(const float* src_proj16, const float* ref_proj16, float* proj12, estd_stream_t stream);

int estd_cam_sweep_proj(const float* ref_pose16, const float* src_pose16, const float* intr9,
                        float* proj12, estd_stream_t stream);

int estd_cam_volume_mats(const float* pose_j16, const float* pose_i16, const float* intr9,
                         float* mats30, estd_stream_t stream);


int estd_homo_warping(const float* src_chw, const float* proj12, const float* depth_values,
                      float* out_cdhw, int C, int D, int H, int W, estd_stream_t stream);

int estd_homo_warping_px(const float* src_chw, const float* proj12, const float* depth_dhw,
                         float* out_cdhw, int C, int D, int H, int W, estd_stream_t stream);

int estd_mix1x1_chw_to_hwc(const float* in_chw, const float* w, const float* bias, float* out_hwc,
                           int Cin, int Cout, int HW, estd_stream_t stream);

int estd_homo_warp_costvol(const float* src_mix_hwc, const float* ref_mix_hwc, const float* proj12,
                           const float* depth_values, float* out_vol32, int D, int H, int W,
                           estd_stream_t stream);

typedef struct estd_conv3d_desc {
    int N, D, H, W;
    int cin_main;
    int in_stride;
    int n_tiles;
    const float* in_main;
    const float* in_extra;
    const float* w_main;
    const float* w_extra;
    const float* w_xout;
    const float* scale;
    const float* shift;
    int act_a, act_b, act_split;
    float* out_main;
    int out_stride;
    int out_channels;
    const float* residual;
    const float* residual2;
    float out_scale;
    int accumulate;
    float* out_extra;
    const float* head_w;
    const float* head_b;
    float* out_head;
    double* stats_partials;
    const void* w_split;
    const float* w_wino;
    const float* w_wino2;
    const float* gate_r;
    const float* gate_stats;
    const float* gate_gamma;
    const float* gate_beta;
} estd_conv3d_desc;

int estd_conv3d_k3(const estd_conv3d_desc* desc, estd_stream_t stream);
#ifdef ESTD_BUILD_AB
int estd_conv3d_k3_split(const estd_conv3d_desc* desc, estd_stream_t stream);
#endif
#ifdef ESTD_BUILD_AB
int estd_conv3d_k3_wino(const estd_conv3d_desc* desc, estd_stream_t stream);
#endif
int estd_conv3d_k3_wino2(const estd_conv3d_desc* desc, estd_stream_t stream);
#ifdef ESTD_BUILD_AB
int estd_conv3d_k3_wino2x(const estd_conv3d_desc* desc, estd_stream_t stream);
#endif
int estd_conv3d_k3_wino3(const estd_conv3d_desc* desc, estd_stream_t stream);
int estd_conv3d_k3_xout(const estd_conv3d_desc* desc, estd_stream_t stream);
int estd_conv3d_k3_grid(int N, int D, int H, int W);

typedef struct estd_conv2d_desc {
    int N, H, W;
    int cin, cout;
    int dilation;
    int group_tiles;
    const float* in;
    const float* w;
    const float* scale;
    const float* shift;
    int relu_before_residual;
    int relu_after_residual;
    const float* residual;
    float* out;
    const void* w_split;
    const float* w_wino;
} estd_conv2d_desc;

int estd_conv2d_k3(const estd_conv2d_desc* desc, estd_stream_t stream);
#ifdef ESTD_BUILD_AB
int estd_conv2d_k3_wino(const estd_conv2d_desc* desc, estd_stream_t stream);
#endif
int estd_conv2d_k3_wino2(const estd_conv2d_desc* desc, estd_stream_t stream);
#ifdef ESTD_BUILD_AB
int estd_conv2d_k3_split(const estd_conv2d_desc* desc, estd_stream_t stream);
#endif

int estd_groupnorm_finalize(const double* partials, int n_blocks, double count, float eps, float* stats_out4,
                            estd_stream_t stream);

int estd_softargmin_up(const float* logits, const float* depth_values, float* depth, float* prob,
                       int N, int D, int H, int W, int s, estd_stream_t stream);


int estd_warp_volume(const float* vol_cdhw, const float* mats30, const float* depth_values,
                     float depth_min, float depth_interval, float* out_cdhw,
                     int C, int D, int H, int W, estd_stream_t stream);

typedef struct estd_warp_volume_opts {
    int depth_per_voxel;
    int use_disp;
    int border;
    float depth_min, depth_interval;
    float disp_min, disp_interval;
    float padding_value;
} estd_warp_volume_opts;
int estd_warp_volume_ex(const float* vol_cdhw, const float* mats30, const float* depth, const estd_warp_volume_opts* opts,
                        float* out_cdhw, int C, int D, int H, int W, estd_stream_t stream);

int estd_warp_attention(const float* kv_target, const float* const* kv_src, const float* mats_dev,
                        int n_src, const float* depth_values, float depth_min, float depth_interval,
                        float* xh_out, int D, int H, int W, estd_stream_t stream);

int estd_attention_prewarped(const float* kv_target, const float* const* kv_src, int n_src,
                             float* xh_out, int64_t n_vox, estd_stream_t stream);

int estd_gru_reset_apply(const float* xh, const float* ru, const float* stats4, const float* gamma_r,
                         const float* beta_r, float* xrh, int64_t n_vox, estd_stream_t stream);

int estd_gru_blend(const float* xh, const float* ru, const float* o_raw, const float* stats_ru4,
                   const float* stats_o4, const float* gamma_u, const float* beta_u, const float* gamma_o,
                   const float* beta_o, float* out_value, int out_stride, int64_t n_vox, estd_stream_t stream);

int estd_cdhw_to_vol(const float* src_cdhw, float* dst, int C, int64_t S, int dst_stride, int dst_off,
                     estd_stream_t stream);
int estd_vol_to_cdhw(const float* src, float* dst_cdhw, int C, int64_t S, int src_stride, int src_off,
                     estd_stream_t stream);

int estd_bn_act_nhwc(float* x, const float* scale, const float* shift, const float* residual, int relu,
                     int64_t n_pix, int C, estd_stream_t stream);

int estd_spp_upsample_cat(const float* raw, int c_raw, const float* skip, int c_skip, const float* const* branches,
                          const int* bh, const int* bw, int nb, int c_b, float* out, int N, int H, int W,
                          estd_stream_t stream);

int estd_conv2d_small_nhwc(const float* in, const float* w_packed, const float* scale, const float* shift, float* out, int N, int Hin,
                           int Win, int cin, int cout, int ksize, int stride, int relu, estd_stream_t stream);
typedef struct estd_conv1x1_desc {
    int N, H, W;
    int cin, cout;
    int stride;
    int relu;
    const float* in;
    const float* w;
    const float* scale;
    const float* shift;
    const float* residual;
    float* out;
} estd_conv1x1_desc;
int estd_conv1x1_nhwc(const estd_conv1x1_desc* desc, estd_stream_t stream);
typedef struct estd_conv2d_taps_desc {
    int N, H, W;
    int cin, cout;
    int ksize, stride, pad;
    int relu;
    const float* in;
    const float* w;
    const float* scale;
    const float* shift;
    const float* residual;
    float* out;
} estd_conv2d_taps_desc;
int estd_conv2d_taps_nhwc(const estd_conv2d_taps_desc* desc, estd_stream_t stream);
int estd_stem7x7s2_nhwc(const float* in, const float* w_packed, const float* scale, const float* shift, float* out, int N, int H,
                        int W, estd_stream_t stream);
int estd_maxpool3x3s2_nhwc(const float* in, float* out, int N, int H, int W, int C, estd_stream_t stream);
int estd_avgpool_nhwc(const float* in, float* out, int N, int H, int W, int C, int k, estd_stream_t stream);
int estd_conv2d_k3_to16_nhwc(const float* in, const float* w_packed, const float* scale, const float* shift, float* out, int N,
                             int H, int W, int cin, int upsample, estd_stream_t stream);
int estd_normalise_nhwc(const float* in, float* out, int N, int64_t HW, estd_stream_t stream);
int estd_stem3x3s2_nhwc(const float* in, const float* w, const float* scale, const float* shift, float* out, int N, int H, int W,
                        estd_stream_t stream);
int estd_planes_cat_nhwc(const float* a, int Ca, const float* b, int Cb, int relu_b, float* out, int N, int64_t HW,
                         estd_stream_t stream);
int estd_nhwc_to_planes(const float* in, int C, float* out, int N, int64_t HW, estd_stream_t stream);
int estd_upsample2_cat_nhwc(const float* x, int Cx, const float* skip, int Cs, float* out, int N, int H, int W,
                            estd_stream_t stream);
int estd_disp_head_nhwc(const float* in, const float* w, const float* bias, float depth_max, float* out, int N, int H, int W,
                        int C, int upscale, estd_stream_t stream);

#define ESTD_TSDF_MAX_FRAMES 8
typedef struct estd_tsdf_integrate_desc {
    int Z, Y, X;
    int T;
    int H, W;
    int weighted;
    int no_skip;
    float trunc, z_near, conf_min, w_max;
    float* tsdf;
    float* weight;
    const float* depth[ESTD_TSDF_MAX_FRAMES];
    const float* conf[ESTD_TSDF_MAX_FRAMES];
    float mats[ESTD_TSDF_MAX_FRAMES][12];
} estd_tsdf_integrate_desc;
int estd_tsdf_integrate(const estd_tsdf_integrate_desc* desc, estd_stream_t stream);

typedef struct estd_tsdf_integrate_color_desc {
    int Z, Y, X;
    int T;
    int H, W;
    int weighted;
    int no_skip;
    float trunc, z_near, conf_min, w_max;
    float* tsdf;
    float* weight;
    const float* depth[ESTD_TSDF_MAX_FRAMES];
    const float* conf[ESTD_TSDF_MAX_FRAMES];
    float mats[ESTD_TSDF_MAX_FRAMES][12];
    float* color;
    const float* image[ESTD_TSDF_MAX_FRAMES];
} estd_tsdf_integrate_color_desc;
int estd_tsdf_integrate_color(const estd_tsdf_integrate_color_desc* desc, estd_stream_t stream);

int estd_tsdf_extract_points(const float* tsdf, const float* weight, int Z, int Y, int X, float voxel_size, const float* origin3,
                             float w_min, unsigned long long* counter, long long capacity, float* xyz, float* normal,
                             float* point_weight, long long* edge, estd_stream_t stream);

int estd_tsdf_edge_colors(const float* tsdf, const float* color, int Z, int Y, int X, const long long* edge, long long n, float* out,
                          estd_stream_t stream);

typedef struct estd_tsdf_raycast_desc {
    int Z, Y, X;
    int H, W;
    int n_steps;
    float t_min, dt;
    float w_min;
    const float* tsdf;
    const float* weight;
    float* depth;
    float* normal;
    float* out_weight;
    unsigned int* stats;
    float mat[12];
} estd_tsdf_raycast_desc;
int estd_tsdf_raycast(const estd_tsdf_raycast_desc* desc, estd_stream_t stream);

typedef struct estd_tsdf_raycast_color_desc {
    int Z, Y, X;
    int H, W;
    int n_steps;
    float t_min, dt;
    float w_min;
    const float* tsdf;
    const float* weight;
    float* depth;
    float* normal;
    float* out_weight;
    unsigned int* stats;
    float mat[12];
    const float* color;
    float* out_color;
} estd_tsdf_raycast_color_desc;
int estd_tsdf_raycast_color(const estd_tsdf_raycast_color_desc* desc, estd_stream_t stream);

#define ESTD_CONSISTENCY_MAX_SOURCES 8
typedef struct estd_depth_consistency_desc {
    int H, W;
    int S;
    float px_max, rel_max, z_near;
    const float* target;
    const float* source[ESTD_CONSISTENCY_MAX_SOURCES];
    float* views;
    float* visible;
    float* depth;
    float* rel_err;
    float mats[ESTD_CONSISTENCY_MAX_SOURCES][2][12];
} estd_depth_consistency_desc;
int estd_depth_consistency(const estd_depth_consistency_desc* desc, estd_stream_t stream);

#define ESTD_CLOUD_KEY_MAX_DIM (1 << 20)
#define ESTD_CLOUD_MAX_DIM 1024
#define ESTD_CLOUD_MAX_CELLS (1 << 24)
#define ESTD_CLOUD_MAX_ATTRS 6
int estd_cloud_cell_keys(const float* points, long long n, const float* lo3, float cell, const int* dims3, long long* keys,
                         estd_stream_t stream);

typedef struct estd_cloud_nearest_desc {
    long long M, N;
    const float* query;
    const long long* order;
    const float* records;
    const int* cell_start;
    float* dist;
    long long* index;
    unsigned int* stats;
    float lo[3];
    float cell;
    float max_dist;
    int dims[3];
} estd_cloud_nearest_desc;
int estd_cloud_nearest(const estd_cloud_nearest_desc* desc, estd_stream_t stream);

int estd_cloud_cell_centroids(const float* points, const float* attrs, int C, long long n, const long long* order,
                              const long long* segments, long long K, float* out_points, float* out_attrs, estd_stream_t stream);

#define ESTD_FRAME_ALIGN_SUMS 29
typedef struct estd_frame_align_desc {
    int H, W;
    int Hm, Wm;
    float dist_max, z_near, conf_min;
    const float* depth;
    const float* conf;
    const float* m_depth;
    const float* m_normal;
    float* residual;
    int* match;
    double* sums;
    double* partials;
    float L[12], Fm[12], Bm[12];
} estd_frame_align_desc;
long long estd_frame_align_partials(int H, int W);
int estd_frame_align(const estd_frame_align_desc* desc, estd_stream_t stream);

int estd_tsdf_mesh_vertices(const float* tsdf, const float* weight, const float* color, int Z, int Y, int X, float voxel_size,
                            const float* origin3, float w_min, unsigned long long* counter, long long capacity, long long* cell,
                            float* xyz, float* normal, float* vertex_weight, float* vertex_color, estd_stream_t stream);
// ... 83 lines not shown
```

Baseline: 199.3 depth frames/s.

## Add split-K across grid for conv2d taps kernel with separate reduce epilogue

Adds a grid-level split-K mode to the NHWC tap convolution. Each y-slice of the grid writes partial sums to a workspace, and a new reduce kernel then applies scale, shift, residual and ReLU. The split factor is chosen from the CU count, the tile count and the chunks per wave, so that small-spatial backbone convs fill the GPU better. The cost is a second launch, a workspace allocation per call and extra global-memory traffic for the partial sums.

Result: no change. 200.0 depth frames/s, median of 6 (+0.3%).

```diff
diff --git a/estdepth_amd/_native.py b/estdepth_amd/_native.py
--- a/estdepth_amd/_native.py
+++ b/estdepth_amd/_native.py
@@ -192,6 +192,9 @@
     "estd_bn_act_nhwc": (ctypes.c_int, [c_float_p, c_float_p, c_float_p, c_float_p, ctypes.c_int, ctypes.c_int64, ctypes.c_int, c_stream]),
     "estd_conv1x1_nhwc": (ctypes.c_int, [ctypes.POINTER(Conv1x1Desc), c_stream]),
     "estd_conv2d_taps_nhwc": (ctypes.c_int, [ctypes.POINTER(Conv2dTapsDesc), c_stream]),
+    "estd_conv2d_taps_ksplit": (ctypes.c_int, [ctypes.POINTER(Conv2dTapsDesc)]),
+    "estd_conv2d_taps_workspace_bytes": (ctypes.c_longlong, [ctypes.POINTER(Conv2dTapsDesc)]),
+    "estd_conv2d_taps_nhwc_ws": (ctypes.c_int, [ctypes.POINTER(Conv2dTapsDesc), ctypes.c_void_p, ctypes.c_size_t, c_stream]),
     "estd_stem7x7s2_nhwc": (ctypes.c_int, [c_float_p, c_float_p, c_float_p, c_float_p, c_float_p, ctypes.c_int, ctypes.c_int, ctypes.c_int, c_stream]),
     "estd_maxpool3x3s2_nhwc": (ctypes.c_int, [c_float_p, c_float_p] + [ctypes.c_int] * 4 + [c_stream]),
     "estd_avgpool_nhwc": (ctypes.c_int, [c_float_p, c_float_p] + [ctypes.c_int] * 5 + [c_stream]),
diff --git a/estdepth_amd/backbones.py b/estdepth_amd/backbones.py
--- a/estdepth_amd/backbones.py
+++ b/estdepth_amd/backbones.py
@@ -158,7 +158,7 @@
         sc, sh = _folded(bn)
         xn = x.contiguous(memory_format=torch.channels_last).permute(0, 2, 3, 1)
         rn = residual.contiguous(memory_format=torch.channels_last).permute(0, 2, 3, 1) if residual is not None else None
-        return ops.conv2d_taps_nhwc(xn, c[1], sc, sh, conv.kernel_size[0], conv.stride[0], conv.padding[0], relu, rn).permute(0, 3, 1, 2)
+        return ops.conv2d_taps_nhwc(xn, c[1], sc, sh, conv.kernel_size[0], conv.stride[0], conv.padding[0], relu, rn, splitk=True).permute(0, 3, 1, 2)
     if GEMM_EPILOGUE and residual is None and _is_1x1(conv) and conv.bias is None:
         return conv1x1_bn_gemm(conv, bn, x, relu)
     y = conv1x1_gemm(conv, x) if _is_1x1(conv) else conv(x)
diff --git a/estdepth_amd/build.py b/estdepth_amd/build.py
--- a/estdepth_amd/build.py
+++ b/estdepth_amd/build.py
@@ -10,7 +10,7 @@
 OBJ_DIR = os.path.join(OUT_DIR, "obj" + os.environ.get("ESTD_LIB_SUFFIX", ""))
 LIB = os.path.join(OUT_DIR, "libestd_hip%s.so" % os.environ.get("ESTD_LIB_SUFFIX", ""))
 SOURCES = ["conv3d_mfma.hip", "conv3d_wino2.hip", "conv3d_wino3.hip", "conv3d_xout.hip", "conv3d_wino2_c16.hip", "conv2d_mfma.hip", "conv2d_wino2.hip",
-           "plane_sweep.hip", "est_fusion.hip", "refine2d.hip", "conv1x1.hip", "conv2d_taps.hip", "tsdf.hip", "tsdf_raycast.hip",
+           "plane_sweep.hip", "est_fusion.hip", "refine2d.hip", "conv1x1.hip", "conv2d_taps.hip", "splitk_reduce.hip", "tsdf.hip", "tsdf_raycast.hip",
            "depth_consistency.hip", "cloud_nn.hip", "track/frame_align.hip", "track/rigid_align.hip",
            "mesh/tsdf_mesh.hip", "mesh/mesh_components.hip",
            "mesh/mesh_sample.hip", "mesh/mesh_raster.hip", "mesh/mesh_distance.hip", "mesh/mesh_simplify.hip"]
diff --git a/estdepth_amd/csrc/conv2d_taps.hip b/estdepth_amd/csrc/conv2d_taps.hip
--- a/estdepth_amd/csrc/conv2d_taps.hip
+++ b/estdepth_amd/csrc/conv2d_taps.hip
@@ -8,8 +8,8 @@
 
 namespace {
 
-template <int TM, int TN, int PF, int SK>
-__global__ __launch_bounds__(256) void conv2d_taps_kernel(const estd_conv2d_taps_desc p, int Ho, int Wo, int tiles_m, int tiles_n)
+template <int TM, int TN, int PF, int SK, bool GS>
+__device__ __forceinline__ void conv2d_taps_body(const estd_conv2d_taps_desc& p, int Ho, int Wo, int tiles_m, int tiles_n, float* __restrict__ ws)
 {
     __shared__ float4 red[SK > 1 ? (SK - 1) * TN * TM * 64 : 1];
     const int lane = threadIdx.x & 63;
@@ -50,8 +50,16 @@
         for (int b = 0; b < TM; ++b) acc[a][b] = (f32x4){0.f, 0.f, 0.f, 0.f};
 
     const int cpt = cin >> 4;
-    const int nchunks = ks * ks * cpt / SK;
-    const int kbase = SK > 1 ? wave * nchunks : 0;
+    int nchunks, kbase;
+    if (GS) {
+        const int total = ks * ks * cpt, S = (int)gridDim.y, s = (int)blockIdx.y;
+        const int g0 = (int)((long long)total * s / S), g1 = (int)((long long)total * (s + 1) / S);
+        const int w0 = g0 + (g1 - g0) * (SK > 1 ? wave : 0) / SK, w1 = g0 + (g1 - g0) * ((SK > 1 ? wave : 0) + 1) / SK;
+        kbase = w0; nchunks = w1 - w0;
+    } else {
+        nchunks = ks * ks * cpt / SK;
+        kbase = SK > 1 ? wave * nchunks : 0;
+    }
     int l_tap = kbase / cpt, l_kc = kbase - l_tap * cpt;
     int l_ky = l_tap / ks, l_kx = l_tap - l_ky * ks;
 
@@ -114,6 +122,21 @@
                     const float4 r = red[((w * TN + a) * TM + b) * 64 + lane];
                     acc[a][b] += (f32x4){r.x, r.y, r.z, r.w};
                 }
+    }
+
+    if (GS) {
+        const __amdgpu_buffer_rsrc_t rs_ws = make_rsrc_bytes(ws + (size_t)blockIdx.y * Mtot * cout, (size_t)Mtot * cout * 4);
+#pragma unroll
+        for (int a = 0; a < TN; ++a)
+#pragma unroll
+            for (int b = 0; b < TM; ++b) {
+                const int m = m0 + 16 * b + i;
+                const unsigned off = m < Mtot ? (unsigned)((size_t)m * cout + n0 + 16 * a + 4 * g) * 4u : OOB_OFFSET;
+                u32x4 bits;
+                __builtin_memcpy(&bits, &acc[a][b], 16);
+                __builtin_amdgcn_raw_buffer_store_b128(bits, rs_ws, off, 0, 0);
+            }
+        return;
     }
 
     const __amdgpu_buffer_rsrc_t rs_o = make_rsrc_bytes(p.out, (size_t)Mtot * cout * 4);
@@ -151,14 +174,32 @@
 }
 
 template <int TM, int TN, int PF, int SK>
-int launch_taps(const estd_conv2d_taps_desc& d, int Ho, int Wo, hipStream_t stream)
+__global__ __launch_bounds__(256) void conv2d_taps_kernel(const estd_conv2d_taps_desc p, int Ho, int Wo, int tiles_m, int tiles_n)
+{
+    conv2d_taps_body<TM, TN, PF, SK, false>(p, Ho, Wo, tiles_m, tiles_n, nullptr);
+}
+
+template <int TM, int TN, int PF, int SK, bool KSPLIT>
+__global__ __launch_bounds__(256) void conv2d_taps_kernel(const estd_conv2d_taps_desc p, int Ho, int Wo, int tiles_m, int tiles_n, float* __restrict__ ws)
+{
+    static_assert(KSPLIT, "the one-launch kernel is the four-argument template");
+    conv2d_taps_body<TM, TN, PF, SK, true>(p, Ho, Wo, tiles_m, tiles_n, ws);
+}
+
+template <int TM, int TN, int PF, int SK>
+int launch_taps(const estd_conv2d_taps_desc& d, int Ho, int Wo, int S, float* ws, hipStream_t stream)
 {
     const long long Mtot = (long long)d.N * Ho * Wo;
     const int tiles_m = (int)((Mtot + 16 * TM - 1) / (16 * TM)), tiles_n = d.cout / (16 * TN);
     const long long wts = (long long)tiles_m * tiles_n;
     const unsigned grid = SK > 1 ? (unsigned)wts : (unsigned)((wts + 3) / 4);
-    hipLaunchKernelGGL((conv2d_taps_kernel<TM, TN, PF, SK>), dim3(grid), dim3(256), 0, stream, d, Ho, Wo, tiles_m, tiles_n);
-    return ESTD_LAUNCH_CHECK();
+    if (S == 1) {
+        hipLaunchKernelGGL((conv2d_taps_kernel<TM, TN, PF, SK>), dim3(grid), dim3(256), 0, stream, d, Ho, Wo, tiles_m, tiles_n);
+        return ESTD_LAUNCH_CHECK();
+    }
+    hipLaunchKernelGGL((conv2d_taps_kernel<TM, TN, PF, SK, true>), dim3(grid, (unsigned)S), dim3(256), 0, stream, d, Ho, Wo, tiles_m, tiles_n, ws);
+    if (ESTD_LAUNCH_CHECK() != ESTD_OK) return ESTD_ERR_LAUNCH;
+    return estd_splitk_reduce_launch(ws, S, Mtot, d.cout, d.scale, d.shift, d.residual, false, d.relu != 0, d.out, stream);
 }
 
 constexpr int STEM_ROWS = 8;
@@ -280,28 +321,49 @@
 
 }
 
-extern "C" int estd_conv2d_taps_nhwc(const estd_conv2d_taps_desc* dp, estd_stream_t s)
-{
-    if (!dp) return ESTD_ERR_ARG;
-    const estd_conv2d_taps_desc& d = *dp;
-    if (d.N <= 0 || d.H <= 0 || d.W <= 0 || !d.in || !d.w || !d.out || d.pad < 0) return ESTD_ERR_ARG;
-    if (d.stride != 1 && d.stride != 2) return ESTD_ERR_UNSUPPORTED;
-    if (d.ksize != 1 && d.ksize != 3 && d.ksize != 5) return ESTD_ERR_UNSUPPORTED;
-    if (d.cin < 16 || (d.cin & 15) || d.cout < 32 || (d.cout & 31)) return ESTD_ERR_UNSUPPORTED;
-    if (d.H + 2 * d.pad < d.ksize || d.W + 2 * d.pad < d.ksize) return ESTD_ERR_ARG;
-    const int Ho = (d.H + 2 * d.pad - d.ksize) / d.stride + 1, Wo = (d.W + 2 * d.pad - d.ksize) / d.stride + 1;
+namespace {
+
+struct taps_plan { int status, Ho, Wo, cfg, S; };
+
+constexpr int TAPS_SPLIT_WAVES_PER_CU = 8;
+constexpr int TAPS_SPLIT_MIN_CHUNKS = 18;
+constexpr int TAPS_SPLIT_MIN = 3;
+constexpr int TAPS_SPLIT_MAX = 8;
+
+taps_plan taps_plan_for(const estd_conv2d_taps_desc& d, bool allow_split)
+{
+    taps_plan pl = {ESTD_OK, 0, 0, 0, 1};
+    if (d.N <= 0 || d.H <= 0 || d.W <= 0 || d.pad < 0) return pl.status = ESTD_ERR_ARG, pl;
+    if (d.stride != 1 && d.stride != 2) return pl.status = ESTD_ERR_UNSUPPORTED, pl;
+    if (d.ksize != 1 && d.ksize != 3 && d.ksize != 5) return pl.status = ESTD_ERR_UNSUPPORTED, pl;
+    if (d.cin < 16 || (d.cin & 15) || d.cout < 32 || (d.cout & 31)) return pl.status = ESTD_ERR_UNSUPPORTED, pl;
+    if (d.H + 2 * d.pad < d.ksize || d.W + 2 * d.pad < d.ksize) return pl.status = ESTD_ERR_ARG, pl;
+    const int Ho = pl.Ho = (d.H + 2 * d.pad - d.ksize) / d.stride + 1, Wo = pl.Wo = (d.W + 2 * d.pad - d.ksize) / d.stride + 1;
     const long long Mtot = (long long)d.N * Ho * Wo;
     const int taps = d.ksize * d.ksize;
     if (((long long)d.N * d.H + d.ksize) * d.W * d.cin * 4 >= 0x7fffff00LL || Mtot * d.cout * 4 >= 0x7fffff00LL ||
         (long long)taps * d.cin * d.cout * 4 >= 0x7fffff00LL)
-        return ESTD_ERR_UNSUPPORTED;
-    hipStream_t stream = estd_stream(s);
+        return pl.status = ESTD_ERR_UNSUPPORTED, pl;
     static const int cfg_env = [] { const char* e = getenv("ESTD_CTAPS_CFG"); return e ? atoi(e) : 0; }();
+    static const int split_env = [] { const char* e = getenv("ESTD_CTAPS_SPLIT"); const int v = e ? atoi(e) : 0; return v < 0 ? 0 : v > 64 ? 64 : v; }();
     const long long want = (long long)estd_device_cus() * 7 / 2;
     auto tiles = [&](int tm, int tn) { return ((Mtot + 16 * tm - 1) / (16 * tm)) * (d.cout / (16 * tn)); };
     const bool sk4 = (d.cin & 63) == 0 && (long long)taps * d.cin >= 256;
     const bool c64 = (d.cout & 63) == 0;
-    int cfg = cfg_env;
+    const int split_cfg = cfg_env ? cfg_env : (c64 ? 440 : 420) + (sk4 ? 4 : 1);
+    if (allow_split && split_env != 1) {
+        pl.S = split_env;
+        if (split_env == 0) {
+            const long long waves = tiles(4, c64 ? 4 : 2) * (sk4 ? 4 : 1);
+            const long long chunks = (long long)taps * (d.cin >> 4) / (sk4 ? 4 : 1);
+            const long long target = (long long)estd_device_cus() * TAPS_SPLIT_WAVES_PER_CU;
+            long long S = target / waves;
+            if (S > chunks / TAPS_SPLIT_MIN_CHUNKS) S = chunks / TAPS_SPLIT_MIN_CHUNKS;
+            if (S > TAPS_SPLIT_MAX) S = TAPS_SPLIT_MAX;
+            pl.S = S < TAPS_SPLIT_MIN ? 1 : (int)S;
+        }
+    }
+    int cfg = pl.S > 1 ? split_cfg : cfg_env;
     if (cfg == 0) {
         if (c64 && tiles(4, 4) >= want) cfg = 441;
         else if (tiles(4, 2) >= want) cfg = 421;
@@ -314,18 +376,63 @@
     }
     if ((cfg % 10) == 4 && (d.cin & 63)) cfg = cfg - 3;
     if ((cfg / 10) % 10 == 4 && !c64) cfg -= 20;
-    switch (cfg) {
-    case 441: return launch_taps<4, 4, 2, 1>(d, Ho, Wo, stream);
-    case 421: return launch_taps<4, 2, 3, 1>(d, Ho, Wo, stream);
-    case 241: return launch_taps<2, 4, 3, 1>(d, Ho, Wo, stream);
-    case 221: return launch_taps<2, 2, 4, 1>(d, Ho, Wo, stream);
-    case 444: return launch_taps<4, 4, 2, 4>(d, Ho, Wo, stream);
-    case 424: return launch_taps<4, 2, 3, 4>(d, Ho, Wo, stream);
-    case 244: return launch_taps<2, 4, 3, 4>(d, Ho, Wo, stream);
-    case 224: return launch_taps<2, 2, 4, 4>(d, Ho, Wo, stream);
-    case 124: return launch_taps<1, 2, 4, 4>(d, Ho, Wo, stream);
-    default: return launch_taps<1, 2, 8, 1>(d, Ho, Wo, stream);
-    }
+    pl.cfg = cfg;
+    return pl;
+}
+
+int taps_launch(const estd_conv2d_taps_desc& d, const taps_plan& pl, float* ws, hipStream_t stream)
+{
+    switch (pl.cfg) {
+    case 441: return launch_taps<4, 4, 2, 1>(d, pl.Ho, pl.Wo, pl.S, ws, stream);
+    case 421: return launch_taps<4, 2, 3, 1>(d, pl.Ho, pl.Wo, pl.S, ws, stream);
+    case 241: return launch_taps<2, 4, 3, 1>(d, pl.Ho, pl.Wo, pl.S, ws, stream);
+    case 221: return launch_taps<2, 2, 4, 1>(d, pl.Ho, pl.Wo, pl.S, ws, stream);
+    case 444: return launch_taps<4, 4, 2, 4>(d, pl.Ho, pl.Wo, pl.S, ws, stream);
+    case 424: return launch_taps<4, 2, 3, 4>(d, pl.Ho, pl.Wo, pl.S, ws, stream);
+    case 244: return launch_taps<2, 4, 3, 4>(d, pl.Ho, pl.Wo, pl.S, ws, stream);
+    case 224: return launch_taps<2, 2, 4, 4>(d, pl.Ho, pl.Wo, pl.S, ws, stream);
+    case 124: return launch_taps<1, 2, 4, 4>(d, pl.Ho, pl.Wo, pl.S, ws, stream);
+    default: return launch_taps<1, 2, 8, 1>(d, pl.Ho, pl.Wo, pl.S, ws, stream);
+    }
+}
+
+long long taps_workspace_bytes(const estd_conv2d_taps_desc& d, const taps_plan& pl)
+{
+    return pl.S > 1 ? (long long)pl.S * d.N * pl.Ho * pl.Wo * d.cout * 4 : 0;
+}
+
+}
+
+extern "C" int estd_conv2d_taps_nhwc(const estd_conv2d_taps_desc* dp, estd_stream_t s)
+{
+    if (!dp || !dp->in || !dp->w || !dp->out) return ESTD_ERR_ARG;
+    const taps_plan pl = taps_plan_for(*dp, false);
+    if (pl.status != ESTD_OK) return pl.status;
+    return taps_launch(*dp, pl, nullptr, estd_stream(s));
+}
+
+extern "C" int estd_conv2d_taps_ksplit(const estd_conv2d_taps_desc* dp)
+{
+    if (!dp) return ESTD_ERR_ARG;
+    const taps_plan pl = taps_plan_for(*dp, true);
+    return pl.status != ESTD_OK ? pl.status : pl.S;
+}
+
+extern "C" long long estd_conv2d_taps_workspace_bytes(const estd_conv2d_taps_desc* dp)
+{
+    if (!dp) return ESTD_ERR_ARG;
+    const taps_plan pl = taps_plan_for(*dp, true);
+    return pl.status != ESTD_OK ? pl.status : taps_workspace_bytes(*dp, pl);
+}
+
+extern "C" int estd_conv2d_taps_nhwc_ws(const estd_conv2d_taps_desc* dp, void* workspace, size_t workspace_bytes, estd_stream_t s)
+{
+    if (!dp || !dp->in || !dp->w || !dp->out) return ESTD_ERR_ARG;
+    const taps_plan pl = taps_plan_for(*dp, true);
+    if (pl.status != ESTD_OK) return pl.status;
+    const long long need = taps_workspace_bytes(*dp, pl);
+    if (need > 0 && (!workspace || (long long)workspace_bytes < need || ((uintptr_t)workspace & 15))) return ESTD_ERR_ARG;
+    return taps_launch(*dp, pl, static_cast<float*>(workspace), estd_stream(s));
 }
 
 extern "C" int estd_stem7x7s2_nhwc(const float* in, const float* w_packed, const float* scale, const float* shift, float* out, int N, int H, int W,
diff --git a/estdepth_amd/csrc/estd_common.h b/estdepth_amd/csrc/estd_common.h
--- a/estdepth_amd/csrc/estd_common.h
+++ b/estdepth_amd/csrc/estd_common.h
@@ -60,6 +60,9 @@
 
 int estd_wino2_c16_launch(const estd_conv3d_desc& d, hipStream_t stream);
 
+int estd_splitk_reduce_launch(const float* workspace, int S, long long pixels, int cout, const float* scale, const float* shift, const float* residual,
+                              bool relu_before, bool relu_after, float* out, hipStream_t stream);
+
 static inline int estd_ceil_div(long long a, long long b) { return (int)((a + b - 1) / b); }
 
 template <auto Kernel>
diff --git a/estdepth_amd/csrc/splitk_reduce.hip b/estdepth_amd/csrc/splitk_reduce.hip
--- /dev/null
+++ b/estdepth_amd/csrc/splitk_reduce.hip
@@ -0,0 +1,49 @@
+#include <hip/hip_runtime.h>
+#include <stdint.h>
+
+#include "estd_hip.h"
+#include "estd_common.h"
+#include "estd_device.h"
+
+namespace {
+
+__global__ __launch_bounds__(256) void conv2d_taps_kernel_reduce_kernel(const float4* __restrict__ ws, int S, long long quads, int c4,
+                                                                        const float4* __restrict__ scale, const float4* __restrict__ shift,
+                                                                        const float4* __restrict__ residual, float floor_before, float floor_after,
+                                                                        float4* __restrict__ out)
+{
+    const long long e = (long long)blockIdx.x * 256 + threadIdx.x;
+    if (e >= quads) return;
+    const int c = (int)(e % c4);
+    float4 acc = ws[e];
+    int s = 1;
+    for (; s + 4 <= S; s += 4) {
+        const float4 p0 = ws[(long long)s * quads + e], p1 = ws[(long long)(s + 1) * quads + e];
+        const float4 p2 = ws[(long long)(s + 2) * quads + e], p3 = ws[(long long)(s + 3) * quads + e];
+        acc = f4_add(f4_add(f4_add(f4_add(acc, p0), p1), p2), p3);
+    }
+    for (; s < S; ++s) acc = f4_add(acc, ws[(long long)s * quads + e]);
+    float4 sc = make_float4(1.f, 1.f, 1.f, 1.f), sh = make_float4(0.f, 0.f, 0.f, 0.f);
+    if (scale) sc = scale[c];
+    if (shift) sh = shift[c];
+    float4 v = make_float4(fmaf(acc.x, sc.x, sh.x), fmaf(acc.y, sc.y, sh.y), fmaf(acc.z, sc.z, sh.z), fmaf(acc.w, sc.w, sh.w));
+    v.x = fmaxf(v.x, floor_before); v.y = fmaxf(v.y, floor_before); v.z = fmaxf(v.z, floor_before); v.w = fmaxf(v.w, floor_before);
+    if (residual) v = f4_add(v, residual[e]);
+    v.x = fmaxf(v.x, floor_after); v.y = fmaxf(v.y, floor_after); v.z = fmaxf(v.z, floor_after); v.w = fmaxf(v.w, floor_after);
+    out[e] = v;
+}
+
+}
+
+int estd_splitk_reduce_launch(const float* workspace, int S, long long pixels, int cout, const float* scale, const float* shift, const float* residual,
+                              bool relu_before, bool relu_after, float* out, hipStream_t stream)
+{
+    if (!workspace || !out || S < 1 || pixels <= 0 || cout <= 0 || (cout & 3)) return ESTD_ERR_ARG;
+    const long long quads = pixels * (cout / 4);
+    const long long blocks = (quads + 255) / 256;
+    if (blocks > 0x7fffffffLL) return ESTD_ERR_ARG;
+    hipLaunchKernelGGL(conv2d_taps_kernel_reduce_kernel, dim3((unsigned)blocks), dim3(256), 0, stream, reinterpret_cast<const float4*>(workspace), S, quads, cout / 4,
+                       reinterpret_cast<const float4*>(scale), reinterpret_cast<const float4*>(shift), reinterpret_cast<const float4*>(residual),
+                       relu_before ? 0.0f : ESTD_NO_FLOOR, relu_after ? 0.0f : ESTD_NO_FLOOR, reinterpret_cast<float4*>(out));
+    return ESTD_LAUNCH_CHECK();
+}
diff --git a/estdepth_amd/csrc/torch_ops.cpp b/estdepth_amd/csrc/torch_ops.cpp
--- a/estdepth_amd/csrc/torch_ops.cpp
+++ b/estdepth_amd/csrc/torch_ops.cpp
@@ -1082,8 +1082,8 @@
     return out;
 }
 
-template <class Desc>
-static Tensor desc_conv(const char* op, int (*launch)(const Desc*, estd_stream_t), const char* what, Desc d, const Tensor& x, const Tensor& w,
+template <class Desc, class Launch>
+static Tensor desc_conv(const char* op, Launch launch, const char* what, Desc d, const Tensor& x, const Tensor& w,
                         at::IntArrayRef w_tail, int64_t ho, int64_t wo, const OptTensor& scale, const OptTensor& shift, bool relu,
                         const OptTensor& residual)
 {
@@ -1122,6 +1122,26 @@
     estd_conv2d_taps_desc d{};
     d.ksize = (int)ksize; d.stride = (int)stride; d.pad = (int)pad;
     return desc_conv(op, estd_conv2d_taps_nhwc, "estd_conv2d_taps_nhwc", d, x, w_taps, {ksize * ksize, -1, x.size(-1)},
+                     (x.size(-3) + 2 * pad - ksize) / stride + 1, (x.size(-2) + 2 * pad - ksize) / stride + 1, scale, shift, relu, residual);
+}
+
+Tensor conv2d_taps_splitk_nhwc(const Tensor& x, const Tensor& w_taps, const OptTensor& scale, const OptTensor& shift, int64_t ksize, int64_t stride,
+                               int64_t pad, bool relu, const OptTensor& residual)
+{
+    const char* op = "conv2d_taps_nhwc";
+    const OpScope scope(x);
+    map_ptr(x, {-1, -1, -1, -1}, op, "x");
+    check_count(stride, 1, 2, op, "stride");
+    estd_conv2d_taps_desc d{};
+    d.ksize = (int)ksize; d.stride = (int)stride; d.pad = (int)pad;
+    Tensor ws;
+    auto launch = [&x, &ws](const estd_conv2d_taps_desc* dp, estd_stream_t stream) -> int {
+        const long long need = estd_conv2d_taps_workspace_bytes(dp);
+        if (need < 0) return (int)need;
+        if (need > 0) ws = new_f32({need / 4}, x);
+        return estd_conv2d_taps_nhwc_ws(dp, need > 0 ? ws.data_ptr<float>() : nullptr, (size_t)need, stream);
+    };
+    return desc_conv(op, launch, "estd_conv2d_taps_nhwc_ws", d, x, w_taps, {ksize * ksize, -1, x.size(-1)},
                      (x.size(-3) + 2 * pad - ksize) / stride + 1, (x.size(-2) + 2 * pad - ksize) / stride + 1, scale, shift, relu, residual);
 }
 
@@ -1478,6 +1498,7 @@
     m.def("spp_upsample_cat(Tensor raw, Tensor skip, Tensor[] branches) -> Tensor");
     m.def("conv1x1_nhwc(Tensor x, Tensor w, Tensor? scale, Tensor? shift, int stride, bool relu, Tensor? residual) -> Tensor");
     m.def("conv2d_taps_nhwc(Tensor x, Tensor w, Tensor? scale, Tensor? shift, int ksize, int stride, int pad, bool relu, Tensor? residual) -> Tensor");
+    m.def("conv2d_taps_splitk_nhwc(Tensor x, Tensor w, Tensor? scale, Tensor? shift, int ksize, int stride, int pad, bool relu, Tensor? residual) -> Tensor");
     m.def("stem7x7s2_nhwc(Tensor x, Tensor w_packed, Tensor scale, Tensor shift) -> Tensor");
     m.def("maxpool3x3s2_nhwc(Tensor x) -> Tensor");
     m.def("avgpool_nhwc(Tensor x, int k) -> Tensor");
@@ -1556,6 +1577,7 @@
     m.impl("spp_upsample_cat", spp_upsample_cat);
     m.impl("conv1x1_nhwc", conv1x1_nhwc);
     m.impl("conv2d_taps_nhwc", conv2d_taps_nhwc);
+    m.impl("conv2d_taps_splitk_nhwc", conv2d_taps_splitk_nhwc);
     m.impl("stem7x7s2_nhwc", stem7x7s2_nhwc);
     m.impl("maxpool3x3s2_nhwc", maxpool3x3s2_nhwc);
     m.impl("avgpool_nhwc", avgpool_nhwc);
diff --git a/estdepth_amd/ops.py b/estdepth_amd/ops.py
--- a/estdepth_amd/ops.py
+++ b/estdepth_amd/ops.py
@@ -760,7 +760,7 @@
     return out
 
 
-def _desc_conv(op, entry, d, x, w, w_tail, ho, wo, scale, shift, relu, residual):
+def _desc_conv(op, entry, d, x, w, w_tail, ho, wo, scale, shift, relu, residual, ws_bytes=None):
     n, h, wd, cin = x.shape[-4:]
     dev = x.device
     cout = _map(w, w_tail, op, "w", dev)[-2]
@@ -772,7 +772,15 @@
         d.residual = residual.data_ptr()
     out = torch.empty((n, ho, wo, cout), device=dev)
     d.out = out.data_ptr()
-    _launch(dev, entry, ctypes.byref(d))
+    if ws_bytes is None:
+        _launch(dev, entry, ctypes.byref(d))
+        return out
+    with torch.cuda.device(dev):
+        need = ws_bytes(ctypes.byref(d))
+    if need < 0:
+        N.check(need, ws_bytes.__name__)
+    ws = torch.empty(need // 4, device=dev) if need else None
+    _launch(dev, entry, ctypes.byref(d), _p(ws), need)
     return out
 
 
@@ -787,17 +795,29 @@
     return _desc_conv(op, N.lib().estd_conv1x1_nhwc, d, x, w2, (-1, c), (h - 1) // stride + 1, (w - 1) // stride + 1, scale, shift, relu, residual)
 
 
-def conv2d_taps_nhwc(x, w_taps, scale, shift, ksize, stride=1, pad=None, relu=False, residual=None):
+def conv2d_taps_nhwc(x, w_taps, scale, shift, ksize, stride=1, pad=None, relu=False, residual=None, splitk=False):
     pad = ksize // 2 if pad is None else pad
     if _use_torch():
-        return T().conv2d_taps_nhwc(x, w_taps, scale, shift, int(ksize), int(stride), int(pad), bool(relu), residual)
+        fn = T().conv2d_taps_splitk_nhwc if splitk else T().conv2d_taps_nhwc
+        return fn(x, w_taps, scale, shift, int(ksize), int(stride), int(pad), bool(relu), residual)
     op = "conv2d_taps_nhwc"
     n, h, w, c = _map(x, (-1, -1, -1, -1), op, "x")
     _count(stride, 1, 2, op, "stride")
     d = N.Conv2dTapsDesc()
     d.ksize, d.stride, d.pad = int(ksize), int(stride), int(pad)
-    return _desc_conv(op, N.lib().estd_conv2d_taps_nhwc, d, x, w_taps, (ksize * ksize, -1, c), (h + 2 * pad - ksize) // stride + 1,
-                      (w + 2 * pad - ksize) // stride + 1, scale, shift, relu, residual)
+    entry, ws_bytes = (N.lib().estd_conv2d_taps_nhwc_ws, N.lib().estd_conv2d_taps_workspace_bytes) if splitk else (N.lib().estd_conv2d_taps_nhwc, None)
+    return _desc_conv(op, entry, d, x, w_taps, (ksize * ksize, -1, c), (h + 2 * pad - ksize) // stride + 1,
+                      (w + 2 * pad - ksize) // stride + 1, scale, shift, relu, residual, ws_bytes)
+
+
+def conv2d_taps_ksplit(n, h, w, cin, cout, ksize, stride=1, pad=None):
+    d = N.Conv2dTapsDesc()
+    d.N, d.H, d.W, d.cin, d.cout = int(n), int(h), int(w), int(cin), int(cout)
+    d.ksize, d.stride, d.pad = int(ksize), int(stride), int(ksize // 2 if pad is None else pad)
+    s = N.lib().estd_conv2d_taps_ksplit(ctypes.byref(d))
+    if s < 0:
+        N.check(s, "estd_conv2d_taps_ksplit")
+    return s
 
 
 def _packed_conv(op, entry, x, w, scale, shift, out_shape, *sizes):
diff --git a/include/estd_hip.h b/include/estd_hip.h
--- a/include/estd_hip.h
+++ b/include/estd_hip.h
@@ -1,6 +1,7 @@
 #ifndef ESTD_HIP_H
 #define ESTD_HIP_H
 
+#include <stddef.h>
 #include <stdint.h>
 
 #ifdef __cplusplus
@@ -200,6 +201,9 @@
     float* out;
 } estd_conv2d_taps_desc;
 int estd_conv2d_taps_nhwc(const estd_conv2d_taps_desc* desc, estd_stream_t stream);
+int estd_conv2d_taps_ksplit(const estd_conv2d_taps_desc* desc);
+long long estd_conv2d_taps_workspace_bytes(const estd_conv2d_taps_desc* desc);
+int estd_conv2d_taps_nhwc_ws(const estd_conv2d_taps_desc* desc, void* workspace, size_t workspace_bytes, estd_stream_t stream);
 int estd_stem7x7s2_nhwc(const float* in, const float* w_packed, const float* scale, const float* shift, float* out, int N, int H,
                         int W, estd_stream_t stream);
 int estd_maxpool3x3s2_nhwc(const float* in, float* out, int N, int H, int W, int C, estd_stream_t stream);
```
